# VIDILabs/open-volume-renderer

Measured on AMD Instinct MI355X. Metric: Msamples/s (primary ray-march samples after ERT); fps alongside, higher is better.
Workload: dtype f32

## Files before the change

open-volume-renderer_amd/csrc/host/frame.cpp:

```cpp
#include "state.hpp"

#include <cstdio>
#include <cstdlib>

namespace ovrhip {
namespace host {

static_assert(policy::kGeneral == LAYOUT_GENERAL && policy::kThin == LAYOUT_THIN && policy::kThinT == LAYOUT_THIN_T && policy::kQuad == LAYOUT_QUAD
              && policy::kLayoutCount == kLayouts && policy::kPoolSubCount == kPoolSubs, "policy.hpp restates ovr_hip_kernels.h");


static void shade_order_params(ovr_hip_renderer* r, PoolDesc& pd)
{
  const float beam = r->shade_beam;
  pd.order_grid = 0;
  if (!r->shade_order_on || !pd.order || !pd.order_key || !pd.order_ws) { pd.order = nullptr; return; }
  const RayMarchParams& P = r->P;
  const double diag = std::sqrt((double)r->vd.nx * r->vd.nx + (double)r->vd.ny * r->vd.ny + (double)r->vd.nz * r->vd.nz);
  const int G = diag <= 32.0 * beam ? 32 : diag <= 64.0 * beam ? 64 : 128;
  const double L[3] = { P.light.x, P.light.y, P.light.z };
  const int k = std::fabs(L[0]) <= std::fabs(L[1]) && std::fabs(L[0]) <= std::fabs(L[2]) ? 0 : std::fabs(L[1]) <= std::fabs(L[2]) ? 1 : 2;
  double U[3] = { 0, 0, 0 }, V[3];
  U[(k + 1) % 3] = L[(k + 2) % 3]; U[(k + 2) % 3] = -L[(k + 1) % 3];
  const double un = std::sqrt(U[0] * U[0] + U[1] * U[1] + U[2] * U[2]);
// ... 156 lines not shown
      HIP_TRY(hipMemsetAsync(r->d_grad[i], 0, n * 3 * sizeof(float), st));
    }
    if (f.recon_on) HIP_TRY(hipMemsetAsync(r->recon.d_count, 0, std::max<size_t>(n, 1) * sizeof(float), st));
  }
  r->frame_index++;
  return 0;
}

static void fill_target_params(ovr_hip_renderer* r, const FrameSetup& f)
{
  RayMarchParams& P = r->P;
  P.rgba = r->d_rgba[r->cur];
  nonzero_rect(r, r->d_rect[r->cur]);
  if (r->shard.current.world > 1 && r->group.members.size() <= 1) r->map_whole_set(r->cur);
  if (f.recon_on) r->map_whole_set(r->cur);
  r->recon.frame = f.recon_on;
  r->frame_set = r->cur;
  P.grad = r->d_grad[r->cur];
  P.accum = r->d_accum;
  P.width = r->fbsize.current.w;
  P.height = r->fbsize.current.h;
  P.frame_index = r->frame_index;
  P.accumulate = f.accumulate ? 1 : 0;
  P.spp = r->spp.current;
  P.shading = r->shading.current;
  P.step = 1.f / r->rate.current;
  P.base = 1.f;
  P.shadow_stride = (P.step * 10.f) * P.step;
  const float ex = r->spacing[0] * r->vd.nx, ey = r->spacing[1] * r->vd.ny, ez = r->spacing[2] * r->vd.nz;
  P.long_ray_steps = std::sqrt(ex * ex + ey * ey + ez * ez) / P.step;
}

static void choose_layout(ovr_hip_renderer* r, hipStream_t st)
{
  RayMarchParams& P = r->P;
  int choice = r->layout_choice.current;
  if (choice < 0) {
    const float dir[3] = { P.cam_dir.x, P.cam_dir.y, P.cam_dir.z }, inv_scale[3] = { P.inv_scale.x, P.inv_scale.y, P.inv_scale.z };
    choice = policy::layout_rule(dir, inv_scale);
  }
  const bool tune_l = r->layout_choice.current < 0, tune_p = r->pipeline.current == 0;
  const bool may_wait = !tune_l;
  if (choice < 0 || choice >= kLayouts || r->replica_state[choice] == 0) choice = LAYOUT_GENERAL;
  bool building = false;
  if (r->tune.on && (tune_l || tune_p) && r->tune.state == 1) {
    int states[kLayouts];
    for (int k = 0; k < kLayouts; ++k) states[k] = r->replica_state[k];
    const int wanted = r->tune.probe_build(tune_l, states);
    if (wanted >= 0) (void)start_replica_build(r, wanted, nullptr);
    building = poll_replica_builds(r) > 0;
    (void)hipGetLastError();
  }
  choice = r->tune.before_frame(choice, tune_l, tune_p, building);
  choice = resolve_layout(r, choice, may_wait, st);
  const float vs = P.vol.value_scale, vm = P.vol.value_min_clamp;
  P.vol = r->vd_replica[choice];
  P.vol.value_scale = vs;
  P.vol.value_min_clamp = vm;
  r->stats.layout = choice;
}

static void bind_general_layout(ovr_hip_renderer* r)
{
  RayMarchParams& P = r->P;
  const float vs = P.vol.value_scale, vm = P.vol.value_min_clamp;
  P.vol = r->vd_replica[LAYOUT_GENERAL];
  P.vol.value_scale = vs;
  P.vol.value_min_clamp = vm;
  r->stats.layout = LAYOUT_GENERAL;
  r->tune.frame = -1;
}

const float* projection_ranges(const ovr_hip_renderer* r) { return r->have_volume && r->mc_ranges_valid ? r->d_mc_minmax : nullptr; }

void fill_isosurface_params(const ovr_hip_renderer* r, RayMarchParams& q)
{
  const IsoP& p = r->isosurfaces.current;
  q.iso_n = p.n;
  for (int k = 0; k < OVR_HIP_MAX_ISOVALUES; ++k) q.iso_values[k] = k < p.n ? p.v[k] : 0.f;
}
static bool in_place_frame(const RayMarchParams& P) { return P.projection != OVR_HIP_PROJECT_OFF || P.iso_n > 0; }

static int fill_table_params(ovr_hip_renderer* r)
{
  RayMarchParams& P = r->P;
  P.tf_color = r->d_tf_color;
  P.tf_alpha = r->d_tf_alpha;
  P.n_color = r->n_color;
  P.n_alpha = r->n_alpha;
  P.rank = r->shard.current.rank;
  P.world = r->shard.current.world;
  P.tile_w = r->shard.current.tw;
  P.tile_h = r->shard.current.th;
  P.lds_staging = r->lds_staging.current;
  P.lds_brick_offset = 0;
  P.jitter_mode = r->jitter.current;
  P.jitter_noise = r->d_noise;
  P.jitter_xy = r->noise_xy;
  if (P.jitter_mode == 1 && !r->d_noise)
    return fail(OVR_HIP_ESTATE, "[hip] blue-noise pixel jitter enabled but no noise tile was set (ovr_hip_set_noise_tile)");
  P.counters = r->d_counters;
  P.majorant = nullptr;
  P.occupancy = nullptr;
  P.occupancy_fine = nullptr;
  P.projection = r->projection.current;
  P.mc_ranges = nullptr;
  fill_isosurface_params(r, P);
  return 0;
}

static int choose_skipping(ovr_hip_renderer* r, FrameSetup& f)
{
  RayMarchParams& P = r->P;
  if (in_place_frame(P)) {
    f.use_skip = false;
    if (r->skipping.current != 0) P.mc_ranges = projection_ranges(r);
  }
  else f.use_skip = r->skip.before_frame(r->skipping.current != 0, r->mc_majorant_valid);
  if (f.use_skip) {
    if (int e = update_macrocells(r, f.st)) return e;
    P.majorant = r->d_mc_majorant;
    P.occupancy = r->d_mc_occupancy;
// ... 266 lines not shown
  f.recon_on = r->reconstruction.current == OVR_HIP_RECONSTRUCT_FILL && f.sparse && r->shard.current.world <= 1 && r->group.members.size() <= 1 && !r->group.leader;
  if (f.recon_on)
    if (int e = ensure_reconstruction(r)) return e;
  if (int e = reset_accumulation(r, f)) return e;
  fill_target_params(r, f);
  if (r->projection.current != OVR_HIP_PROJECT_OFF || r->isosurfaces.current.n > 0) bind_general_layout(r);
  else choose_layout(r, st);
  if (int e = fill_table_params(r)) return e;
  if (int e = choose_skipping(r, f)) return e;
  r->P.shadow_lattice = nullptr;
  if (!in_place_frame(r->P) && r->P.shading == OVR_HIP_SHADE_FULL && r->shadow.current.mode != OVR_HIP_SHADOWS_MARCHED)
    if (int e = ensure_shadow_cache(r, r->P, st)) return e;
  f.conv_on = r->convergence.current.mode != OVR_HIP_CONVERGENCE_OFF && f.accumulate && !f.sparse;
  r->P.accum_half = nullptr;
  r->P.conv_asked = nullptr;
  if (f.conv_on) {
    if (int e = ensure_convergence(r, false)) return e;
    r->P.accum_half = r->conv.d_accum_half;
  }
  if (!f.sparse)
    if (int e = schedule_blocks(r, f)) return e;
  if (int e = prepare_convergence(r, f)) return e;
  if (r->conv.resolve_only) return launch_frame(r);
  if (f.sparse)
    if (int e = launch_frame_mask(r, f)) return e;
  if (int e = prepare_pool(r, f)) return e;
  return launch_frame(r);
}

static int launch_frame(ovr_hip_renderer* r)
{
  hipStream_t st = r->stream();
  const bool resolve = r->P.accum_half && r->convergence.current.mode == OVR_HIP_CONVERGENCE_ADAPTIVE && r->conv.retired > 0;
  const int blocks_x = (r->fbsize.current.w + 7) / 8;
  if (r->conv.resolve_only) {
    HIP_TRY(hipEventRecord(r->ev[0], st));
    HIP_TRY(launch_resolve_blocks(r->P, r->conv.d_lists + r->conv.list_cap, r->conv.retired, r->conv.d_frames, r->conv.d_grad_keep, blocks_x, st));
    HIP_TRY(hipEventRecord(r->ev[3], st));
    std::memset(r->h_counters, 0, 8 * sizeof(unsigned long long));
    r->frame_phase_timed = false;
    r->async_pending = true;
    return 0;
  }
  if (resolve) HIP_TRY(launch_resolve_blocks(r->P, r->conv.d_lists + r->conv.list_cap, r->conv.retired, r->conv.d_frames, r->conv.d_grad_keep, blocks_x, st));
  r->P.publish = r->h_counters;
  r->P.reduce_done = reinterpret_cast<unsigned int*>(reinterpret_cast<char*>(r->d_counters) + 128 + (size_t)kPoolCtrlWords * sizeof(unsigned int));
  r->P.zero_first = r->frame_words_dirty ? 1 : 0;
  if (r->frame_words_dirty) HIP_TRY(hipMemsetAsync(r->P.reduce_done, 0, sizeof(unsigned int), st));
  if (r->frame_words_dirty && r->pool.order_ws) HIP_TRY(hipMemsetAsync(r->pool.order_ws, 0, (size_t)kOrderWsWords * sizeof(unsigned int), st));
  r->frame_words_dirty = true;
  const bool phases = r->phase_timing.load();
  hipEvent_t evs[4] = { r->ev[0], phases ? r->ev[1] : nullptr, phases ? r->ev[2] : nullptr, r->ev[3] };
  r->frame_phase_timed = phases;
  r->plan = plan_raymarch(r->P);
  HIP_TRY(launch_raymarch(r->P, r->plan, st, evs));
  r->frame_words_dirty = false;
  if (r->conv.frame) {
    ConvergenceParams c{};
    c.accum = r->d_accum; c.accum_half = r->conv.d_accum_half; c.grad = r->P.grad; c.grad_keep = r->conv.d_grad_keep;
    c.width = r->P.width; c.height = r->P.height; c.frame_index = r->P.frame_index;
    c.rank = r->P.rank; c.world = r->P.world; c.tile_w = r->P.tile_w; c.tile_h = r->P.tile_h;
    c.blocks_x = blocks_x;
    c.adaptive = r->convergence.current.mode == OVR_HIP_CONVERGENCE_ADAPTIVE ? 1 : 0;
    c.threshold = r->convergence.current.threshold;
    c.sorted = r->conv.sorted; c.n_work = r->sched.n_work;
    c.active = r->P.schedule; c.n_active = r->P.n_schedule;
    c.active_out = r->conv.d_lists; c.retired_out = r->conv.d_lists ? r->conv.d_lists + r->conv.list_cap : nullptr;
    c.counts = r->conv.d_lists ? r->conv.d_lists + 2 * r->conv.list_cap : nullptr;
    c.block_error = r->conv.d_error; c.block_frames = r->conv.d_frames; c.words = r->conv.d_words;
    c.sub_capacity = r->P.pool.reqs ? r->P.pool.sub_capacity : 0xffffffffu;
    c.publish = r->conv.h_publish;
    r->conv.h_publish[3] = 0u;
    HIP_TRY(launch_convergence(c, st));
  }
  if (r->recon.frame) {
    ReconParams& c = r->recon.params;
    c = ReconParams{};
    c.width = r->P.width; c.height = r->P.height;
    (void)recon_plan(c);
    c.rgba = r->P.rgba; c.grad = r->P.grad;
    c.count = r->recon.d_count;
    c.accum = r->P.accumulate ? r->d_accum : nullptr;
    c.grad_sum = r->P.accumulate ? r->recon.d_grad : nullptr;
    c.pyramid = r->recon.d_pyramid;
    c.words = r->recon.d_words;
    c.sub_capacity = r->P.pool.reqs ? r->P.pool.sub_capacity : 0xffffffffu;
    c.publish = r->recon.h_publish;
    c.frame_index = r->P.frame_index;
    r->recon.h_publish[1] = 0u;
    r->recon.timed = phases;
    if (phases) HIP_TRY(hipEventRecord(r->recon.ev[0], st));
    HIP_TRY(launch_recon_scatter(c, r->recon.d_count, r->P.accumulate ? r->recon.d_grad : nullptr, r->P.sparse_xy, r->P.sparse_count, st));
    HIP_TRY(launch_reconstruct(c, st));
    if (phases) HIP_TRY(hipEventRecord(r->recon.ev[1], st));
  }
  r->async_pending = true;
  return 0;
}

static int resolve_pool(ovr_hip_renderer* r)
{
  if (r->P.pool.reqs) {
    auto asked = [&]() { return (size_t)r->h_ctrl[32 * (kPoolSubs + 1)]; };
    if (asked() > r->pool.sub_capacity && r->packed_early) r->stats.stale_tiles = 1;
    for (int attempt = 0; attempt < 4 && asked() > r->pool.sub_capacity; ++attempt) {
      if (int e = ensure_pool(r, policy::pool_grown(asked()))) return e;
      r->P.pool = r->pool;
      shade_order_params(r, r->P.pool);
// ... 165 lines not shown
```

open-volume-renderer_amd/csrc/host/launch_plan.hpp:

```cpp
#pragma once

#include <algorithm>
#include <cstddef>

namespace ovrhip {

constexpr int kBlock = 256;
constexpr int kWaves = kBlock / 64;
constexpr int request_queue_entries(int shade, bool pooled) { return shade == 0 ? 0 : (pooled ? 128 : 256); }
template <int SHADE, bool POOLED> struct QCfg {
  static constexpr int K = POOLED ? 4 : (SHADE == 0 ? 4 : 3);
  static constexpr int QCAP = request_queue_entries(SHADE, POOLED);
};
constexpr int kShadeReqBytes = 32;
constexpr int kLdsBrickCap = 384;
constexpr int kLdsRegionBytes = 32;
constexpr int kShadeBlocks = 1024;
constexpr unsigned int kDeepMaxBlocks = 10000;
constexpr int kCounterWords = 8;
constexpr int kAxisAbExtra = 3, kAxisZExtra = 2;

constexpr bool row_load_layout(int elem_bytes, bool quad) { return elem_bytes <= 2 && !quad; }
constexpr bool march_variant_exists(int shade, int am, bool pooled, bool skip, bool lds_staged, bool deep, bool material, bool clipped, bool f32_general,
                                    bool cached = false)
{
  if (cached && !(shade == 1 && material && !pooled)) return false;
  if (shade < 0 || shade > 2 || am < 0 || am > 4 || (f32_general && am == 4)) return false;
  if (pooled && shade == 0) return false;
  if (lds_staged) return f32_general && shade == 0 && !skip && am <= 1 && !deep && !material && !clipped;
  if (deep) return pooled && !skip && (am <= 1 || am == 4) && !material && !clipped;
  if (material && (shade == 0 || pooled)) return false;
  if (clipped && !pooled && material != (shade != 0)) return false;
  return true;
}
constexpr bool shade_variant_exists(int shade, int am, bool skip, bool material, bool clipped, bool cached = false)
{
  if (shade < 1 || shade > 2 || am < 0 || am > 4) return false;
  if (cached && !(shade == 1 && material)) return false;
  (void)skip;
  return !clipped || (shade == 2 && material);
}

constexpr int kProjectMaximum = 1, kProjectMinimum = 2, kProjectMean = 3;
constexpr int kProjectK = 4;
constexpr bool project_variant_exists(int mode, int am, bool skip, bool clipped)
{
  (void)clipped;
  if (mode < kProjectMaximum || mode > kProjectMean || am < 0 || am > 4) return false;
  return !skip || mode != kProjectMean;
}

constexpr int kMaxIsovalues = 4;
constexpr bool isosurface_variant_exists(int shade, int am, bool skip, bool clipped)
{
  (void)skip; (void)clipped;
  return shade >= 0 && shade <= 2 && am >= 0 && am <= 4;
}

constexpr size_t tf_lds_bytes(int n_color, int n_alpha)
{
  const size_t need = (size_t)n_color * 16 + (size_t)n_alpha * 4 + 32;
  return need <= 96 * 1024 ? need : 0;
}
constexpr size_t axis_table_bytes(int nx, int ny, int nz, int am)
{
  const size_t ab = (size_t)(nx + ny + kAxisAbExtra), ez = (size_t)(nz + kAxisZExtra);
  return am == 3 ? 0 : am == 2 ? ez * 8 + ab * 4 : (ab + ez) * 4;
}
constexpr size_t align16(size_t n) { return (n + 15) & ~(size_t)15; }

constexpr int addressing_mode(unsigned long long stored_bytes, int elem_bytes, int nx, int ny, int nz, int n_color, int n_alpha)
{
  const int am = stored_bytes <= 0x100000000ull ? 0 : (stored_bytes / (unsigned long long)elem_bytes < 0xffffffffull) ? 1 : 2;
  const size_t tables = axis_table_bytes(nx, ny, nz, am);
  const size_t fixed = tf_lds_bytes(n_color, n_alpha) + (size_t)kWaves * request_queue_entries(1, false) * kShadeReqBytes + 1024;
  return ((am == 2 && tables > 64 * 1024) || tables + 16 + fixed > 160 * 1024) ? 3 : am;
}

struct LaunchFacts {
  int elem_bytes = 4;
  bool quad = false, f32_general = false;
  int nx = 1, ny = 1, nz = 1;
  unsigned long long stored_bytes = 0;
  bool tables = true;
  int n_color = 1, n_alpha = 1, shading = 0;
  bool pool = false, skipping = false, sparse = false;
  unsigned long long sparse_hint_pixels = 0;
  int world = 1;
  unsigned int n_blocks_owned = 0, n_schedule = 0;
  bool schedule = true;
  bool clip_on = false, lds_staging = false;
  int row_loads = 0;
  int shade_blocks = 0;
  bool reference_material = true, shade_order = false;
  bool shadow_cache = false;
  int projection = 0;
  bool ranges = false;
  int isosurfaces = 0;
};
struct LaunchOverrides { int addressing = -1, deep = -1, shade_blocks = 0; };

struct LaunchPlan {
  int shading = 0;
  int am = 0;
  bool pooled = false, skip = false;
  struct March { bool lds_staged = false, deep = false, material = false, clipped = false; } march;
  struct Shade { bool material = false, clipped = false; } shade;
  bool shade_order = false;
  bool cached = false;
  struct Project { int mode = 0; bool skip = false, clipped = false; size_t lds_bytes = 0; } project;
  struct Isosurface { bool on = false, skip = false, clipped = false; size_t lds_bytes = 0; } isosurface;
  size_t march_lds_bytes = 0, shade_lds_bytes = 0;
  unsigned int lds_brick_offset = 0;
  int shade_grid_blocks = 0;
  bool error = false;
};

inline bool deep_rounds_pay(const LaunchFacts& f, const LaunchOverrides& o)
{
  if (o.deep >= 0) return o.deep != 0;
  if (f.sparse) return f.world == 1 && f.sparse_hint_pixels > 0 && f.sparse_hint_pixels <= 64ull * kDeepMaxBlocks;
  return f.world > 1 && f.n_blocks_owned <= kDeepMaxBlocks;
}

inline LaunchPlan plan_projection(const LaunchFacts& f, const LaunchOverrides& o)
{
  LaunchPlan pl;
  int am = addressing_mode(f.stored_bytes, f.elem_bytes, f.nx, f.ny, f.nz, f.n_color, f.n_alpha);
  if (o.addressing >= 0) am = std::min(std::max(am, o.addressing), 3);
  if (f.projection < kProjectMaximum || f.projection > kProjectMean || f.quad || (am < 3 && !f.tables) || (!f.sparse && f.n_schedule > 0 && !f.schedule)) {
    pl.error = true;
    return pl;
  }
  if (row_load_layout(f.elem_bytes, f.quad) && am == 0 && (f.row_loads > 0 ? f.row_loads != 1 : f.stored_bytes > (128ull << 20))) am = 4;
  pl.am = am;
  pl.project.mode = f.projection;
  pl.project.skip = f.ranges && f.projection != kProjectMean;
  pl.project.clipped = f.clip_on;
  pl.project.lds_bytes = std::max<size_t>(align16(axis_table_bytes(f.nx, f.ny, f.nz, am)), (size_t)kWaves * kCounterWords * 4);
  pl.march_lds_bytes = pl.project.lds_bytes;
  return pl;
}

inline LaunchPlan plan_isosurface(const LaunchFacts& f, const LaunchOverrides& o)
{
  LaunchPlan pl;
  int am = addressing_mode(f.stored_bytes, f.elem_bytes, f.nx, f.ny, f.nz, f.n_color, f.n_alpha);
  if (o.addressing >= 0) am = std::min(std::max(am, o.addressing), 3);
  if (f.isosurfaces < 1 || f.isosurfaces > kMaxIsovalues || f.quad || (am < 3 && !f.tables) || (!f.sparse && f.n_schedule > 0 && !f.schedule)) {
    pl.error = true;
    return pl;
  }
  if (row_load_layout(f.elem_bytes, f.quad) && am == 0 && (f.row_loads > 0 ? f.row_loads != 1 : f.stored_bytes > (128ull << 20))) am = 4;
  pl.am = am;
  pl.shading = f.shading == 0 || f.shading == 1 ? f.shading : 2;
  pl.isosurface.on = true;
  pl.isosurface.skip = f.ranges;
  pl.isosurface.clipped = f.clip_on;
  pl.isosurface.lds_bytes = std::max<size_t>(align16(axis_table_bytes(f.nx, f.ny, f.nz, am)), (size_t)kWaves * kCounterWords * 4);
  pl.march_lds_bytes = pl.isosurface.lds_bytes;
  return pl;
}

inline LaunchPlan plan_launch(const LaunchFacts& f, const LaunchOverrides& o = LaunchOverrides())
{
  if (f.isosurfaces != 0) return plan_isosurface(f, o);
  if (f.projection != 0) return plan_projection(f, o);
  LaunchPlan pl;
  pl.shading = f.shading == 0 || f.shading == 1 ? f.shading : 2;
  pl.cached = pl.shading == 2 && f.shadow_cache;
  if (pl.cached) pl.shading = 1;
  const int sh = pl.shading;
  int am = addressing_mode(f.stored_bytes, f.elem_bytes, f.nx, f.ny, f.nz, f.n_color, f.n_alpha);
  if (o.addressing >= 0) am = std::min(std::max(am, o.addressing), 3);
  const size_t tf = tf_lds_bytes(f.n_color, f.n_alpha);
  if ((am < 3 && !f.tables) || tf == 0 || (!f.sparse && f.n_schedule > 0 && !f.schedule)) { pl.error = true; return pl; }
  if (row_load_layout(f.elem_bytes, f.quad) && am == 0 && (f.row_loads > 0 ? f.row_loads != 1 : f.stored_bytes > (128ull << 20))) am = 4;
  pl.am = am;
  pl.skip = f.skipping;
  pl.pooled = sh != 0 && f.pool;
  const size_t tables = align16(axis_table_bytes(f.nx, f.ny, f.nz, am));
  const size_t queues = (size_t)kWaves * request_queue_entries(sh, pl.pooled) * kShadeReqBytes;
  if (!pl.pooled) {
    pl.march_lds_bytes = std::max<size_t>(tf + tables + queues, (size_t)kWaves * kCounterWords * 4);
    if (f.f32_general && sh == 0 && !f.skipping && am <= 1 && f.lds_staging && !f.sparse && !f.clip_on) {
      pl.march.lds_staged = true;
      pl.lds_brick_offset = (unsigned int)align16(pl.march_lds_bytes);
      pl.march_lds_bytes = pl.lds_brick_offset + (size_t)kLdsBrickCap * 128 + kLdsRegionBytes + 12 * 4 + 2 * 4 + 16;
    }
    else {
      pl.march.clipped = f.clip_on;
      pl.march.material = sh != 0 && (f.clip_on || !f.reference_material || pl.cached);
    }
    return pl;
  }
  pl.march_lds_bytes = queues + tables + (size_t)f.n_alpha * 4 + 64;
  pl.march.clipped = f.clip_on;
  pl.march.deep = !f.skipping && (am <= 1 || am == 4) && !f.clip_on && deep_rounds_pay(f, o);
  pl.shade.clipped = sh == 2 && f.clip_on;
  pl.shade.material = pl.shade.clipped || !f.reference_material || pl.cached;
  pl.shade_order = sh == 2 && f.shade_order;
  pl.shade_lds_bytes = std::max<size_t>(tf + tables, 64);
  const int blocks = o.shade_blocks > 0 ? o.shade_blocks : f.shade_blocks;
  pl.shade_grid_blocks = blocks > 0 ? std::min(blocks, kShadeBlocks) : kShadeBlocks;
  return pl;
}

}
```

open-volume-renderer_amd/csrc/host/state.hpp:

```cpp
#pragma once

#include "../../../include/ovr_hip.h"
#include "../ovr_hip_kernels.h"
#include "../ovr_hip_update.h"
#pragma GCC visibility push(hidden)
#include "commit_plan.hpp"
#include "policy.hpp"
#pragma GCC visibility pop

#include <hip/hip_runtime.h>

#include <algorithm>
#include <atomic>
#include <cmath>
#include <cstdint>
#include <cstring>
#include <functional>
#include <mutex>
#include <string>
#include <thread>
#include <vector>

struct ovr_hip_renderer;
struct GroupWorker;
// ... 115 lines not shown
  bool shipped_by_rccl = false;
  float* d_payload[2] = { nullptr, nullptr };
  float* d_gather[2] = { nullptr, nullptr };
  size_t payload_floats[2] = { 0, 0 }, stride[2] = { 0, 0 };
  int fb[5] = { 0, 0, 0, 0, 0 };
  bool grad = true;
  void* rccl_comm = nullptr;
  ovr_hip_stats own_stats{};
  double gather_ms = 0.0;
  double upload_ms = 0.0;
  double update_ms = 0.0;
  GroupWorker* worker = nullptr;
  hipEvent_t ev_gathered = nullptr;
  bool broken = false;
  std::string broken_why;
  double host_us[4] = { 0, 0, 0, 0 };
};

}
}

struct ovr_hip_renderer {
  template <typename T> using Queued = ovrhip::host::Queued<T>;
  int device = 0;
  std::mutex mtx;
  hipStream_t own_stream[2] = { nullptr, nullptr };
  hipStream_t user_stream = nullptr;
  bool use_user_stream = false;
  hipEvent_t ev[4] = { nullptr, nullptr, nullptr, nullptr };

  Queued<ovrhip::host::Size2> fbsize;
  Queued<ovrhip::host::CameraP> camera;
  Queued<ovrhip::host::TfnP> tfn;
  Queued<ovrhip::host::FocusP> focus;
  Queued<int> spp, sparse, accumulate, shading, grid_convention, pipeline, skipping, jitter, lds_staging;
  Queued<int> projection;
  bool projection_skipped = false;
  Queued<ovrhip::host::IsoP> isosurfaces;
  bool isosurface_skipped = false;
  Queued<float> rate;
  Queued<ovrhip::host::ShardP> shard;
  Queued<ovrhip::host::LightP> light;
  Queued<ovrhip::host::MaterialP> material;
  Queued<ovrhip::host::ClipP> clip;
  Queued<ovrhip::host::ShadowP> shadow;
  Queued<ovrhip::host::ConvP> convergence;
  Queued<int> reconstruction;
  Queued<int> layouts;
  Queued<int> layout_choice;

  void* d_volume = nullptr;
  std::atomic<size_t> volume_bytes{ 0 };
  ovrhip::VolumeDesc vd{};
  void* d_replica[ovrhip::kLayouts] = {};
  void* d_axis[ovrhip::kLayouts] = {};
  ovrhip::VolumeDesc vd_replica[ovrhip::kLayouts] = {};
  std::atomic<int> replica_state[ovrhip::kLayouts] = {};
  std::thread builder[ovrhip::kLayouts];
  hipStream_t build_stream = nullptr;
  hipEvent_t build_ev[ovrhip::kLayouts] = {};
  int value_type = 0;
  float origin[3] = { 0, 0, 0 }, spacing[3] = { 1, 1, 1 };
  bool have_volume = false;
  float data_lower = 0.f, data_upper = 0.f;
  float* d_data_range = nullptr;
  double upload_ms[4] = { 0, 0, 0, 0 };
  void* d_update_stage = nullptr;
  size_t update_stage_bytes = 0;
  double update_ms[4] = { 0, 0, 0, 0 };

  ovrhip::policy::Tuner tune;
  ovrhip::policy::AutoPipeline auto_pipe;
  ovrhip::policy::Skip skip;
  bool shade_order_on = true;
  float shade_beam = 32.f;

  float* d_mc_minmax = nullptr;
  float* d_mc_majorant = nullptr;
  unsigned char* d_mc_occupancy = nullptr;
  unsigned char* d_mc_fine = nullptr;
  size_t mc_cells = 0;
  bool mc_ranges_valid = false, mc_majorant_valid = false;

  float* d_tf_color = nullptr;
  float* d_tf_alpha = nullptr;
  float* h_tf = nullptr;
  hipEvent_t ev_tf = nullptr;
  bool tf_copy_pending = false;
  int n_color = 0, n_alpha = 0;
  bool have_tfn = false;

  float* d_rgba[2] = { nullptr, nullptr };
  float* d_grad[2] = { nullptr, nullptr };
  float* h_rgba[2] = { nullptr, nullptr };
  float* h_grad[2] = { nullptr, nullptr };
  int h_rgba_rect[2][4] = {}, h_grad_rect[2][4] = {};
  int d_rect[2][4] = {};
  float* d_accum = nullptr;
  uint32_t* d_rgba8 = nullptr;
  uint32_t* h_rgba8 = nullptr;
  uint16_t* d_rgba16f = nullptr;
  uint16_t* h_rgba16f = nullptr;
  float* d_spp_rgba = nullptr;
  float* d_spp_grad = nullptr;
  size_t fb_pixels = 0;
  int cur = 0;
  bool fb_reset = true;
  int frame_index = 0;
  bool camera_dirty = true;

  ovrhip::host::ConvergenceState conv;
  ovrhip::host::ReconstructionState recon;
  ovrhip::host::ShadowCacheState shadow_cache;

  float* d_noise = nullptr;
  int noise_xy = 0;
  int32_t* d_sparse_xy = nullptr;
  unsigned int* d_block_counts = nullptr;
  unsigned long long* d_sparse_count = nullptr;
  size_t sparse_pixels = 0;
  unsigned long long sparse_prev_pixels = 0;

  unsigned long long* d_counters = nullptr;
  std::atomic<bool> phase_timing{ true };
  bool frame_phase_timed = true;
  bool frame_words_dirty = true;
  unsigned int* d_block_counters = nullptr;
// ... 81 lines not shown
```

open-volume-renderer_amd/csrc/host/update_extent.hpp:

```cpp
#pragma once

#include <algorithm>
#include <cstdint>

namespace ovrhip {
namespace update {

struct Box { int lo[3], hi[3]; };

struct Geometry { int cx, mbx, by, bz; bool transposed, quad; int lx, ly, lz; };

enum { kOk = 0, kNull = 1, kMemKind = 2, kType = 3, kExtent = 4, kOutside = 5 };
inline int check_arguments(const void* data, const int32_t* lower, const int32_t* extent, int mem_kind, int value_type, int resident_type, const int dims[3])
{
  if (!data || !lower || !extent) return kNull;
  if (mem_kind != 0 && mem_kind != 1) return kMemKind;
  if (value_type != resident_type) return kType;
  for (int k = 0; k < 3; ++k)
    if (extent[k] < 1) return kExtent;
  for (int k = 0; k < 3; ++k)
    if (lower[k] < 0 || lower[k] >= dims[k] || extent[k] > dims[k] - lower[k]) return kOutside;
  return kOk;
}
inline const char* check_text(int rule)
{
  switch (rule) {
  case kNull: return "null argument";
  case kMemKind: return "bad mem_kind";
  case kType: return "value_type is not the resident volume's";
  case kExtent: return "extent must be positive";
  case kOutside: return "the box leaves the grid";
  default: return "";
  }
}

struct BrickRange {
  int brick_lo, brick_hi;
  int macro_lo, macro_hi;
  int row_lo, row_hi;
  int layer_lo, layer_hi;
};

inline void pair_axis_bricks(int cx, int na, int bricks_total, int a, int b, int& lo, int& hi)
{
  const int p_lo = a == 0 ? 0 : a + 1;
  lo = p_lo == 0 ? 0 : (p_lo - 1) / cx;
  hi = b == na ? bricks_total - 1 : std::min(b / cx, bricks_total - 1);
}

inline BrickRange brick_range(const Geometry& g, const int dims[3], int macros_a, const Box& box)
{
  const int ia = g.transposed ? 1 : 0, ib = g.transposed ? 0 : 1;
  BrickRange r;
  pair_axis_bricks(g.cx, dims[ia], macros_a * g.mbx, box.lo[ia], box.hi[ia], r.brick_lo, r.brick_hi);
  r.macro_lo = r.brick_lo / g.mbx; r.macro_hi = r.brick_hi / g.mbx;
  r.row_lo = box.lo[ib] >> 5; r.row_hi = (box.hi[ib] - 1) >> 5;
  r.layer_lo = box.lo[2] >> g.bz; r.layer_hi = (box.hi[2] - 1) >> g.bz;
  return r;
}

struct QuadRange {
  int u_lo, u_hi, v_lo, v_hi;
  int macro_lo, macro_hi;
  int row_lo, row_hi;
  int layer_lo, layer_hi;
};
inline QuadRange quad_range(const Geometry& g, const Box& box)
{
  QuadRange r;
  r.u_lo = box.lo[0]; r.u_hi = box.hi[0];
  r.v_lo = box.lo[1]; r.v_hi = box.hi[1];
  r.macro_lo = r.u_lo >> 5; r.macro_hi = r.u_hi >> 5;
  r.row_lo = r.v_lo >> 5; r.row_hi = r.v_hi >> 5;
  r.layer_lo = box.lo[2] >> g.lz; r.layer_hi = (box.hi[2] - 1) >> g.lz;
  return r;
}

inline void macrocell_axis(int n, int a, int b, int& lo, int& hi)
{
  const int cells = (n + 15) / 16;
  lo = a <= 16 ? 0 : a >> 4;
  hi = std::min(b >> 4, cells - 1);
}
struct CellRange { int lo[3], hi[3]; };
inline CellRange macrocell_range(const int dims[3], const Box& box)
{
  CellRange c;
  for (int k = 0; k < 3; ++k) macrocell_axis(dims[k], box.lo[k], box.hi[k], c.lo[k], c.hi[k]);
  return c;
}

}
}
```

open-volume-renderer_amd/csrc/host/volume.cpp:

```cpp
#include "state.hpp"

#include <cfloat>
#include <chrono>
#include <cstdlib>

using namespace ovrhip;
using namespace ovrhip::host;

namespace ovrhip {
namespace host {

static float integer_normalize(float value, int type)
{
  switch (type) {
  case OVR_HIP_TYPE_UINT8: return (float)(uint8_t)value / 255.f;
  case OVR_HIP_TYPE_INT8: { const float n = (float)(int8_t)value / 127.f; return n < -1.f ? -1.f : n; }
  case OVR_HIP_TYPE_UINT16: return (float)(uint16_t)value / 65535.f;
  case OVR_HIP_TYPE_INT16: { const float n = (float)(int16_t)value / 32767.f; return n < -1.f ? -1.f : n; }
  case OVR_HIP_TYPE_UINT32: return (float)(uint32_t)value / (float)UINT32_MAX;
  case OVR_HIP_TYPE_INT32: { const float n = (float)(int32_t)value / (float)INT32_MAX; return n < -1.f ? -1.f : n; }
  default: return value;
  }
}
static int device_value_type(int t)
// ... 159 lines not shown
  for (int i = 0; i < na; ++i) a[i] = t.alphas[2 * i + 1];
  HIP_TRY(hipMemcpyAsync(r->d_tf_color, r->h_tf, words * sizeof(float), hipMemcpyHostToDevice, r->stream()));
  if (!r->ev_tf) HIP_TRY(hipEventCreateWithFlags(&r->ev_tf, hipEventDisableTiming));
  HIP_TRY(hipEventRecord(r->ev_tf, r->stream()));
  r->tf_copy_pending = true;
  r->have_tfn = true;
  return 0;
}

static int update_macrocell_ranges(ovr_hip_renderer* r, hipStream_t st)
{
  const size_t cells = (size_t)((r->vd.nx + 15) / 16) * ((r->vd.ny + 15) / 16) * ((r->vd.nz + 15) / 16);
  if (cells != r->mc_cells || !r->d_mc_minmax) {
    HIP_TRY(hipDeviceSynchronize());
    if (r->d_mc_minmax) HIP_TRY(hipFree(r->d_mc_minmax));
    if (r->d_mc_majorant) HIP_TRY(hipFree(r->d_mc_majorant));
    if (r->d_mc_occupancy) HIP_TRY(hipFree(r->d_mc_occupancy));
    if (r->d_mc_fine) HIP_TRY(hipFree(r->d_mc_fine));
    r->d_mc_fine = nullptr;
    r->d_mc_minmax = r->d_mc_majorant = nullptr;
    r->d_mc_occupancy = nullptr;
    r->mc_cells = 0;
    HIP_TRY(hipMalloc((void**)&r->d_mc_minmax, cells * 2 * sizeof(float)));
    HIP_TRY(hipMalloc((void**)&r->d_mc_majorant, cells * sizeof(float)));
    HIP_TRY(hipMalloc((void**)&r->d_mc_occupancy, cells));
    HIP_TRY(hipMalloc((void**)&r->d_mc_fine, cells));
    r->mc_cells = cells;
    r->mc_ranges_valid = r->mc_majorant_valid = false;
  }
  if (!r->mc_ranges_valid) {
    VolumeDesc vd = r->vd;
    vd.data = r->d_volume;
    HIP_TRY(launch_macrocell_ranges(vd, r->d_mc_minmax, st));
    r->mc_ranges_valid = true;
    r->mc_majorant_valid = false;
  }
  return 0;
}

int update_macrocells(ovr_hip_renderer* r, hipStream_t st)
{
  if (int e = update_macrocell_ranges(r, st)) return e;
  const size_t cells = r->mc_cells;
  if (!r->mc_majorant_valid) {
    HIP_TRY(launch_macrocell_majorants(r->d_mc_minmax, (unsigned int)cells, r->d_tf_alpha, r->n_alpha, r->P.tf_lower, r->P.tf_upper, r->d_mc_majorant, st));
    HIP_TRY(launch_macrocell_coarse(r->d_mc_majorant, r->vd.nx, r->vd.ny, r->vd.nz, r->d_mc_occupancy, r->d_mc_fine, st));
    r->mc_majorant_valid = true;
  }
  return 0;
}

void join_builders(ovr_hip_renderer* r)
{
  for (int k = 0; k < kLayouts; ++k)
    if (r->builder[k].joinable()) r->builder[k].join();
}

static void drop_replica(ovr_hip_renderer* r, int k)
{
  if (k == LAYOUT_GENERAL) return;
  if (r->builder[k].joinable()) r->builder[k].join();
  if (r->d_replica[k]) { (void)hipFree(r->d_replica[k]); r->volume_bytes -= (size_t)r->vd_replica[k].bytes; }
  if (r->d_axis[k]) (void)hipFree(r->d_axis[k]);
  r->d_replica[k] = nullptr; r->d_axis[k] = nullptr;
  r->replica_state[k] = 0;
}

static void build_replica_host(ovr_hip_renderer* r, int k, std::string* err)
{
  (void)hipSetDevice(r->device);
  VolumeDesc t = r->vd_replica[k];
  void *d_data = nullptr, *d_tab = nullptr;
  hipError_t e = hipMalloc(&d_data, (size_t)t.bytes + 64);
  if (e == hipSuccess) e = hipMalloc(&d_tab, axis_table_bytes(t));
  if (e == hipSuccess) {
    t.data = d_data;
    if (getenv("OVR_HIP_POISON_ALLOC") && atoi(getenv("OVR_HIP_POISON_ALLOC")) != 0) e = hipMemsetAsync(d_data, 0xff, (size_t)t.bytes, r->build_stream);
    if (e == hipSuccess) e = hipMemsetAsync((char*)d_data + (size_t)t.bytes, 0, 64, r->build_stream);
  }
  if (e == hipSuccess) e = launch_axis_tables(t, d_tab, r->build_stream);
  if (e == hipSuccess) {
    VolumeDesc g = r->vd_replica[LAYOUT_GENERAL];
    g.data = r->d_volume;
    e = launch_rebrick(g, d_data, t, r->build_stream);
  }
  if (e == hipSuccess) e = hipEventRecord(r->build_ev[k], r->build_stream);
  if (e != hipSuccess) {
    (void)hipGetLastError();
    (void)hipStreamSynchronize(r->build_stream);
    if (err) *err = hipGetErrorString(e);
    if (d_data) (void)hipFree(d_data);
    if (d_tab) (void)hipFree(d_tab);
    r->replica_state[k].store(0, std::memory_order_release);
    return;
  }
  r->vd_replica[k] = t;
  r->d_replica[k] = d_data;
  r->d_axis[k] = d_tab;
  r->volume_bytes += (size_t)t.bytes;
  r->replica_state[k].store(2, std::memory_order_release);
}

int start_replica_build(ovr_hip_renderer* r, int k, std::string* err, bool background)
{
  int planned = 1;
  if (!r->replica_state[k].compare_exchange_strong(planned, 4)) return 0;
  if (r->builder[k].joinable()) r->builder[k].join();
  static const bool threads = !(getenv("OVR_HIP_BUILD_THREAD") && atoi(getenv("OVR_HIP_BUILD_THREAD")) == 0);
  bool started = false;
  if (background && threads) {
    try { r->builder[k] = std::thread(build_replica_host, r, k, nullptr); started = true; }
    catch (const std::exception&) { started = false; }
  }
  if (!started) build_replica_host(r, k, err);
  return 0;
}

int resolve_layout(ovr_hip_renderer* r, int choice, bool may_wait, hipStream_t st)
{
  if (choice <= LAYOUT_GENERAL || choice >= kLayouts || r->replica_state[choice].load(std::memory_order_acquire) == 0) return LAYOUT_GENERAL;
  if (r->replica_state[choice] == 1) (void)start_replica_build(r, choice, nullptr, !may_wait);
  if (r->replica_state[choice] == 4 && may_wait && r->builder[choice].joinable()) r->builder[choice].join();
  int state = r->replica_state[choice].load(std::memory_order_acquire);
  if (state == 2 && hipEventQuery(r->build_ev[choice]) == hipSuccess) { r->replica_state[choice] = 3; state = 3; }
  if (state == 3) return choice;
  if (state == 2 && may_wait && hipStreamWaitEvent(st, r->build_ev[choice], 0) == hipSuccess) return choice;
  (void)hipGetLastError();
  return LAYOUT_GENERAL;
}
int poll_replica_builds(ovr_hip_renderer* r)
{
  int building = 0;
  for (int k = 1; k < kLayouts; ++k) {
    int state = r->replica_state[k].load(std::memory_order_acquire);
    if (state == 2 && hipEventQuery(r->build_ev[k]) == hipSuccess) { r->replica_state[k] = 3; state = 3; }
    if (state == 2 || state == 4) building++;
  }
  return building;
}

static double ms_since(std::chrono::high_resolution_clock::time_point t0) { return std::chrono::duration<double, std::milli>(std::chrono::high_resolution_clock::now() - t0).count(); }

static int plan_replicas(ovr_hip_renderer* r, int vt, const VolumeDesc& vd)
{
  {
    std::lock_guard<std::mutex> lk(r->mtx);
    (void)r->layouts.update();
  }
  {
    size_t free_b = 0, total_b = 0;
    HIP_TRY(hipMemGetInfo(&free_b, &total_b));
    double planned = 0.0;
    auto plan = [&](int k, VolumeDesc& t) { t = vd; t.data = nullptr; t.axis_ab = nullptr; t.axis_z = nullptr; return volume_layout(replica_voxel_type(vt, k), vd.nx, vd.ny, vd.nz, t); };
    if (r->layouts.current != 0 && replica_voxel_type(vt, LAYOUT_THIN) >= 0) {
      VolumeDesc t1, t2;
      if (plan(LAYOUT_THIN, t1) && plan(LAYOUT_THIN_T, t2) && layout_offsets_fit(t1) && layout_offsets_fit(t2) && (r->layouts.current == 2 || (double)(t1.bytes + t2.bytes) <= 0.4 * (double)free_b)) {
        r->vd_replica[LAYOUT_THIN] = t1; r->vd_replica[LAYOUT_THIN_T] = t2;
        r->replica_state[LAYOUT_THIN] = r->replica_state[LAYOUT_THIN_T] = 1;
        planned += (double)(t1.bytes + t2.bytes);
      }
      else if (r->layouts.current == 2) return fail(OVR_HIP_EINVAL, "[hip] volume replicas requested (layouts mode 2) but one z layer of a thin replica exceeds 2^32 elements");
    }
    static const bool want_quad = !(getenv("OVR_HIP_QUAD") && atoi(getenv("OVR_HIP_QUAD")) == 0);
    if (want_quad && r->layouts.current != 0 && replica_voxel_type(vt, LAYOUT_QUAD) >= 0) {
      VolumeDesc tq;
      if (plan(LAYOUT_QUAD, tq) && layout_offsets_fit(tq) && (r->layouts.current == 2 || (double)tq.bytes + planned <= 0.4 * (double)free_b)) {
        r->vd_replica[LAYOUT_QUAD] = tq;
        r->replica_state[LAYOUT_QUAD] = 1;
      }
    }
  }
  return 0;
}

struct UploadTimes { double alloc = 0.0, copy = 0.0, kern = 0.0; };

static int upload_voxels(ovr_hip_renderer* r, const void* data, int mem_kind, int value_type, std::chrono::high_resolution_clock::time_point t_seg, UploadTimes& t)
{
  const VolumeDesc& vd = r->vd_replica[0];
  hipStream_t st = r->own_stream[0];
  auto relayout_all = [&](const void* src, int z0, int nzc) -> hipError_t {
    return launch_relayout(src, value_type, r->d_replica[0], r->vd_replica[0], z0, nzc, st);
  };

  const size_t in_es = value_type_size(value_type);
  const size_t slice_bytes = (size_t)vd.nx * vd.ny * in_es;
  int src_device = r->device;
  if (mem_kind == OVR_HIP_MEM_DEVICE) {
    hipPointerAttribute_t attr{};
    if (hipPointerGetAttributes(&attr, data) == hipSuccess) src_device = attr.device;
    else (void)hipGetLastError();
  }
  if (mem_kind == OVR_HIP_MEM_DEVICE && src_device == r->device) {
    for (int z0 = 0; z0 < vd.nz; z0 += 32768) {
      const int nzc = std::min(32768, vd.nz - z0);
      HIP_TRY(relayout_all((const char*)data + (size_t)z0 * slice_bytes, z0, nzc));
    }
    HIP_TRY(hipStreamSynchronize(st));
    t.kern += ms_since(t_seg);
  }
  else {
    size_t slab = std::max<size_t>(1, ((size_t)1 << 30) / std::max<size_t>(1, slice_bytes));
    slab = std::min<size_t>(slab, (size_t)vd.nz);
    void* d_stage = nullptr;
    t_seg = std::chrono::high_resolution_clock::now();
    HIP_TRY(hipMalloc(&d_stage, slab * slice_bytes));
    t.alloc += ms_since(t_seg);
    for (int z0 = 0; z0 < vd.nz; z0 += (int)slab) {
      const int nzc = (int)std::min<size_t>(slab, (size_t)(vd.nz - z0));
      t_seg = std::chrono::high_resolution_clock::now();
      hipError_t e = mem_kind == OVR_HIP_MEM_DEVICE
                         ? hipMemcpyPeerAsync(d_stage, r->device, (const char*)data + (size_t)z0 * slice_bytes, src_device, (size_t)nzc * slice_bytes, st)
                         : hipMemcpyAsync(d_stage, (const char*)data + (size_t)z0 * slice_bytes, (size_t)nzc * slice_bytes, hipMemcpyHostToDevice, st);
      if (e == hipSuccess) e = hipStreamSynchronize(st);
      t.copy += ms_since(t_seg);
      t_seg = std::chrono::high_resolution_clock::now();
      if (e == hipSuccess) e = relayout_all(d_stage, z0, nzc);
      if (e == hipSuccess) e = hipStreamSynchronize(st);
      t.kern += ms_since(t_seg);
      if (e != hipSuccess) { (void)hipFree(d_stage); return fail(OVR_HIP_EDEVICE, std::string("[hip] volume upload failed: ") + hipGetErrorString(e)); }
    }
    HIP_TRY(hipFree(d_stage));
  }
  return 0;
}

static int set_volume_one(ovr_hip_renderer* r, const void* data, int mem_kind, int value_type, const int32_t dims[3],
                          const float grid_origin[3], const float grid_spacing[3])
{
  const auto t_call = std::chrono::high_resolution_clock::now();
  UploadTimes t;
  if (!r || !data || !dims || !grid_origin || !grid_spacing) return fail(OVR_HIP_EINVAL, "[hip] ovr_hip_set_volume: null argument");
  for (double& v : r->upload_ms) v = 0.0;
  if (dims[0] < 1 || dims[1] < 1 || dims[2] < 1) return fail(OVR_HIP_EINVAL, "[hip] ovr_hip_set_volume: dims must be positive");
  const int vt = device_voxel_type(value_type);
  if (vt < 0) return fail(OVR_HIP_EINVAL, "[Optix7] unexpected volume type ...");
  if (mem_kind != OVR_HIP_MEM_HOST && mem_kind != OVR_HIP_MEM_DEVICE) return fail(OVR_HIP_EINVAL, "[hip] ovr_hip_set_volume: bad mem_kind");
  if (int e = set_device(r)) return e;
  if (int e = finish_frame_one(r)) return e;
  HIP_TRY(hipDeviceSynchronize());

  hipStream_t st = r->own_stream[0];
  VolumeDesc vd{};
  if (!volume_layout(vt, dims[0], dims[1], dims[2], vd)) return fail(OVR_HIP_EINVAL, "[hip] ovr_hip_set_volume: no layout for this voxel type");
  vd.value_scale = 1.f;
  vd.value_min_clamp = -FLT_MAX;
  if (vt == VOX_U8) vd.value_scale = 1.f / 255.f;
  if (vt == VOX_I8) { vd.value_scale = 1.f / 127.f; vd.value_min_clamp = -127.f; }
  const size_t bytes = (size_t)vd.bytes;
  if (!layout_offsets_fit(vd))
    return fail(OVR_HIP_EINVAL, "[hip] ovr_hip_set_volume: one z layer of the volume exceeds 2^32 stored voxels (x * y too large for the 32-bit in-plane offsets)");

  auto t_seg = std::chrono::high_resolution_clock::now();
  join_builders(r);
  HIP_TRY(hipStreamSynchronize(r->build_stream));
  for (int k = 0; k < kLayouts; ++k) {
    if (r->d_replica[k]) HIP_TRY(hipFree(r->d_replica[k]));
    r->d_replica[k] = nullptr;
    if (r->d_axis[k]) HIP_TRY(hipFree(r->d_axis[k]));
    r->d_axis[k] = nullptr;
    r->vd_replica[k] = VolumeDesc{};
    r->replica_state[k] = 0;
  }
  r->d_volume = nullptr;
  r->have_volume = false;
  HIP_TRY(hipMalloc(&r->d_replica[0], bytes + 64));
  if (getenv("OVR_HIP_POISON_ALLOC") && atoi(getenv("OVR_HIP_POISON_ALLOC")) != 0) HIP_TRY(hipMemsetAsync(r->d_replica[0], 0xff, bytes, st));
  HIP_TRY(hipMemsetAsync((char*)r->d_replica[0] + bytes, 0, 64, st));
  r->d_volume = r->d_replica[0];
  r->volume_bytes = bytes;
  vd.data = r->d_volume;
  r->vd_replica[0] = vd;
  r->replica_state[0] = 3;
  if (int e = plan_replicas(r, vt, vd)) return e;
  HIP_TRY(hipMalloc(&r->d_axis[0], axis_table_bytes(r->vd_replica[0])));
  t.alloc += ms_since(t_seg);
  t_seg = std::chrono::high_resolution_clock::now();
  HIP_TRY(launch_axis_tables(r->vd_replica[0], r->d_axis[0], st));
  vd = r->vd_replica[0];
  if (int e = upload_voxels(r, data, mem_kind, value_type, t_seg, t)) return e;
  t_seg = std::chrono::high_resolution_clock::now();
  r->vd = vd;
  if (r->layouts.current == 2) {
    for (int k = 1; k < kLayouts; ++k) {
      if (r->replica_state[k] != 1) continue;
      std::string err;
      (void)start_replica_build(r, k, &err, false);
      if (r->replica_state[k] != 2) {
        for (int j = 1; j < kLayouts; ++j) drop_replica(r, j);
        return fail(OVR_HIP_EDEVICE, std::string("[hip] volume replicas requested (layouts mode 2) but their allocation failed: ") + err);
      }
    }
    HIP_TRY(hipStreamSynchronize(r->build_stream));
    for (int k = 1; k < kLayouts; ++k)
      if (r->replica_state[k] == 2) r->replica_state[k] = 3;
  }
  r->value_type = value_type;
  std::memcpy(r->origin, grid_origin, sizeof(r->origin));
  std::memcpy(r->spacing, grid_spacing, sizeof(r->spacing));
  r->have_volume = true;
  {
    commit::Changes ch;
    ch.happened(commit::kVolumeUpload);
    commit::CommitFacts facts;
    facts.volume = true;
    apply_effects(r, commit::plan_commit(ch, facts));
  }
  if (int e = update_macrocell_ranges(r, st)) return e;
  HIP_TRY(launch_minmax_reduce(r->d_mc_minmax, (unsigned long long)r->mc_cells, r->d_data_range, st));
  float dr[2] = { 0.f, 0.f };
  HIP_TRY(hipMemcpyAsync(dr, r->d_data_range, sizeof(dr), hipMemcpyDeviceToHost, st));
  HIP_TRY(hipStreamSynchronize(st));
  r->data_lower = dr[0];
  r->data_upper = dr[1];
  r->P.tf_lower = dr[0];
  r->P.tf_upper = dr[1];
  update_tfn_range(r);
  t.kern += ms_since(t_seg);
  r->upload_ms[0] = ms_since(t_call); r->upload_ms[1] = t.alloc; r->upload_ms[2] = t.copy; r->upload_ms[3] = t.kern;
  return 0;
}

static int update_volume_one(ovr_hip_renderer* r, const void* data, int mem_kind, int value_type, const int32_t lower[3], const int32_t extent[3])
{
  const auto t_call = std::chrono::high_resolution_clock::now();
  UploadTimes t;
  for (double& v : r->update_ms) v = 0.0;
  if (int e = set_device(r)) return e;
  if (int e = finish_frame_one(r)) return e;
  hipStream_t st = r->own_stream[0];
  update::Box box;
  for (int k = 0; k < 3; ++k) { box.lo[k] = lower[k]; box.hi[k] = lower[k] + extent[k]; }

  join_builders(r);
  for (int k = 1; k < kLayouts; ++k)
    if (r->replica_state[k].load(std::memory_order_acquire) == 2) HIP_TRY(hipStreamWaitEvent(st, r->build_ev[k], 0));

  const size_t in_es = value_type_size(value_type);
  const size_t slice_bytes = (size_t)extent[0] * (size_t)extent[1] * in_es;
  int src_device = r->device;
  if (mem_kind == OVR_HIP_MEM_DEVICE) {
    hipPointerAttribute_t attr{};
    if (hipPointerGetAttributes(&attr, data) == hipSuccess) src_device = attr.device;
    else (void)hipGetLastError();
  }
  const bool direct = mem_kind == OVR_HIP_MEM_DEVICE && src_device == r->device;
  size_t slab = (size_t)extent[2];
  if (!direct) {
    slab = std::min<size_t>(std::max<size_t>(1, ((size_t)1 << 30) / std::max<size_t>(1, slice_bytes)), (size_t)extent[2]);
    if (r->update_stage_bytes < slab * slice_bytes) {
      const auto t_seg = std::chrono::high_resolution_clock::now();
      if (r->d_update_stage) HIP_TRY(hipFree(r->d_update_stage));
      r->d_update_stage = nullptr; r->update_stage_bytes = 0;
      HIP_TRY(hipMalloc(&r->d_update_stage, slab * slice_bytes));
      r->update_stage_bytes = slab * slice_bytes;
      t.alloc += ms_since(t_seg);
    }
  }
  auto write = [&]() -> int {
    for (int z0 = 0; z0 < extent[2]; z0 += (int)slab) {
      const int nzc = (int)std::min<size_t>(slab, (size_t)(extent[2] - z0));
      const void* src = (const char*)data + (size_t)z0 * slice_bytes;
      auto t_seg = std::chrono::high_resolution_clock::now();
      if (!direct) {
        HIP_TRY(mem_kind == OVR_HIP_MEM_DEVICE ? hipMemcpyPeerAsync(r->d_update_stage, r->device, src, src_device, (size_t)nzc * slice_bytes, st)
                                               : hipMemcpyAsync(r->d_update_stage, src, (size_t)nzc * slice_bytes, hipMemcpyHostToDevice, st));
        HIP_TRY(hipStreamSynchronize(st));
        t.copy += ms_since(t_seg);
        t_seg = std::chrono::high_resolution_clock::now();
        src = r->d_update_stage;
      }
      update::Box part = box;
      part.lo[2] = box.lo[2] + z0; part.hi[2] = part.lo[2] + nzc;
      HIP_TRY(launch_update_general(src, value_type, r->d_replica[0], r->vd_replica[0], part, st));
      if (!direct) HIP_TRY(hipStreamSynchronize(st));
      t.kern += ms_since(t_seg);
    }
    const auto t_seg = std::chrono::high_resolution_clock::now();
    VolumeDesc g = r->vd_replica[LAYOUT_GENERAL];
    g.data = r->d_volume;
    for (int k = 1; k < kLayouts; ++k) {
      const int state = r->replica_state[k].load(std::memory_order_acquire);
      if (state == 2 || state == 3) HIP_TRY(launch_update_replica(g, r->d_replica[k], r->vd_replica[k], box, st));
    }
    const int dims[3] = { r->vd.nx, r->vd.ny, r->vd.nz };
    VolumeDesc vd = r->vd;
    vd.data = r->d_volume;
    HIP_TRY(launch_macrocell_ranges_box(vd, r->d_mc_minmax, update::macrocell_range(dims, box), st));
    HIP_TRY(launch_minmax_reduce(r->d_mc_minmax, (unsigned long long)r->mc_cells, r->d_data_range, st));
    float dr[2] = { 0.f, 0.f };
    HIP_TRY(hipMemcpyAsync(dr, r->d_data_range, sizeof(dr), hipMemcpyDeviceToHost, st));
    HIP_TRY(hipStreamSynchronize(st));
    r->data_lower = dr[0];
    r->data_upper = dr[1];
    r->P.tf_lower = dr[0];
    r->P.tf_upper = dr[1];
    update_tfn_range(r);
    t.kern += ms_since(t_seg);
    return 0;
  };
  if (!r->d_mc_minmax || !r->mc_ranges_valid) return fail(OVR_HIP_ESTATE, "[hip] ovr_hip_update_volume: the resident volume has no macrocell ranges");
  if (int e = write()) {
    r->have_volume = false;
    return e;
  }
  commit::Changes ch;
  ch.happened(commit::kVolumeUpdate);
  commit::CommitFacts facts;
  facts.volume = true;
  apply_effects(r, commit::plan_commit(ch, facts));
  r->update_ms[0] = ms_since(t_call); r->update_ms[1] = t.alloc; r->update_ms[2] = t.copy; r->update_ms[3] = t.kern;
  return 0;
}

}
}

extern "C" {

int ovr_hip_update_volume(ovr_hip_renderer* r, const void* data, int mem_kind, int value_type, const int32_t lower[3], const int32_t extent[3])
{
  if (!r) return fail(OVR_HIP_EINVAL, "[hip] ovr_hip_update_volume: null argument");
  if (!r->have_volume && data && lower && extent) return fail(OVR_HIP_ESTATE, "[hip] ovr_hip_update_volume: no volume is set");
  const int dims[3] = { r->vd.nx, r->vd.ny, r->vd.nz };
  if (const int rule = update::check_arguments(data, lower, extent, mem_kind, value_type, r->value_type, dims))
    return fail(OVR_HIP_EINVAL, std::string("[hip] ovr_hip_update_volume: ") + update::check_text(rule));
  if (r->group.members.size() <= 1) return update_volume_one(r, data, mem_kind, value_type, lower, extent);
  const auto t0 = std::chrono::high_resolution_clock::now();
  if (int e = set_device(r)) return e;
  if (int e = finish_frame(r)) return e;
  const int e = group_call(r, [=](ovr_hip_renderer* m) { return update_volume_one(m, data, mem_kind, value_type, lower, extent); },
                           [&] { return update_volume_one(r, data, mem_kind, value_type, lower, extent); });
  if (e) {
    const std::string msg = g_last_error;
// ... 81 lines not shown
```

open-volume-renderer_amd/csrc/ovr_hip_api.cpp:

```cpp
#include "host/state.hpp"

#include <chrono>
#include <cstdio>
#include <cstdlib>

using namespace ovrhip;
using namespace ovrhip::host;

#define GROUP_FORWARD(r, call)                                                                                          \
  do {                                                                                                                  \
    for (size_t i_ = 1; i_ < (r)->group.members.size(); ++i_) {                                                         \
      ovr_hip_renderer* m = (r)->group.members[i_];                                                                     \
      if (int e_ = (call)) { (void)hipSetDevice((r)->device); return e_; }                                              \
    }                                                                                                                   \
    if ((r)->group.members.size() > 1) (void)hipSetDevice((r)->device);                                                 \
  } while (0)

extern "C" {

const char* ovr_hip_last_error(void) { return g_last_error.c_str(); }
int ovr_hip_abi_version(void) { return OVR_HIP_ABI_VERSION; }

int ovr_hip_create(ovr_hip_renderer** out, int device_id)
{
  if (!out) return fail(OVR_HIP_EINVAL, "[hip] ovr_hip_create: null output pointer");
  *out = nullptr;
  int count = 0;
  if (hipGetDeviceCount(&count) != hipSuccess || count <= 0)
    return fail(OVR_HIP_EDEVICE, "[hip] no HIP device available - this backend has no CPU fallback");
  if (device_id < 0 || device_id >= count) return fail(OVR_HIP_EINVAL, "[hip] invalid device ordinal " + std::to_string(device_id));
  HIP_TRY(hipSetDevice(device_id));
  hipDeviceProp_t prop;
  HIP_TRY(hipGetDeviceProperties(&prop, device_id));
  if (std::string(prop.gcnArchName).find("gfx950") == std::string::npos)
    return fail(OVR_HIP_EDEVICE, std::string("[hip] device is ") + prop.gcnArchName + ", this library is built for gfx950 (MI355X) only");
  ovr_hip_renderer* r = new ovr_hip_renderer();
  r->device = device_id;
  apply_lighting(r);
  apply_clip_box(r);
  auto acquire = [&]() -> int {
    HIP_TRY(hipStreamCreate(&r->own_stream[0]));
    HIP_TRY(hipStreamCreate(&r->own_stream[1]));
    for (int i = 0; i < 4; ++i) HIP_TRY(hipEventCreate(&r->ev[i]));
    {
      int lo = 0, hi = 0;
      if (hipDeviceGetStreamPriorityRange(&lo, &hi) != hipSuccess) { (void)hipGetLastError(); lo = hi = 0; }
      HIP_TRY(hipStreamCreateWithPriority(&r->build_stream, hipStreamNonBlocking, hi));
    }
    for (int k = 0; k < kLayouts; ++k) HIP_TRY(hipEventCreateWithFlags(&r->build_ev[k], hipEventDisableTiming));
    HIP_TRY(hipMalloc((void**)&r->d_counters, kFrameWordsBytes));
    HIP_TRY(hipMemset(r->d_counters, 0, kFrameWordsBytes));
    HIP_TRY(hipMalloc((void**)&r->d_sparse_count, sizeof(unsigned long long)));
    HIP_TRY(hipMalloc((void**)&r->d_data_range, minmax_reduce_floats() * sizeof(float)));
    HIP_TRY(hipHostMalloc((void**)&r->h_counters, 8 * sizeof(unsigned long long) + (size_t)kPoolCtrlWords * sizeof(unsigned int), hipHostMallocDefault));
    r->h_ctrl = reinterpret_cast<unsigned int*>(r->h_counters + 8);
    return 0;
  };
  if (int e = acquire()) { ovr_hip_destroy(r); return e; }
  std::memset(r->h_counters, 0, 8 * sizeof(unsigned long long) + (size_t)kPoolCtrlWords * sizeof(unsigned int));
  r->spp.init(1);
  r->sparse.init(0);
  r->accumulate.init(0);
  r->shading.init(OVR_HIP_SHADE_FULL);
  r->grid_convention.init(OVR_HIP_GRID_CELL_CENTRED);
  r->rate.init(1.f);
  r->layouts.init(1);
  r->layout_choice.init(-1);
  if (const char* f = getenv("OVR_HIP_LAYOUTS")) r->layouts.init(atoi(f));
  if (const char* f = getenv("OVR_HIP_SKIP_ADAPTIVE")) r->skip.adaptive = atoi(f) != 0;
  if (const char* f = getenv("OVR_HIP_TUNE")) r->tune.on = atoi(f) != 0;
  if (const char* f = getenv("OVR_HIP_SHADE_ORDER")) r->shade_order_on = atoi(f) != 0;
  if (const char* f = getenv("OVR_HIP_ROW_LOADS")) r->P.row_loads = atoi(f) != 0 ? 2 : 1;
  if (const char* f = getenv("OVR_HIP_SHADE_BEAM")) r->shade_beam = std::max(1.f, (float)atof(f));
  *out = r;
  return 0;
}
void ovr_hip_destroy(ovr_hip_renderer* r)
{
  if (!r) return;
  if (r->group.members.size() > 1) group_stop_workers(r);
  for (size_t i = 1; i < r->group.members.size(); ++i) ovr_hip_destroy(r->group.members[i]);
  r->group.members.clear();
  join_builders(r);
  (void)hipSetDevice(r->device);
  (void)hipDeviceSynchronize();
  group_release(r);
  (void)free_framebuffers(r);
  for (int k = 0; k < kLayouts; ++k) {
    if (r->d_replica[k]) (void)hipFree(r->d_replica[k]);
    if (r->d_axis[k]) (void)hipFree(r->d_axis[k]);
  }
  if (r->d_tf_color) (void)hipFree(r->d_tf_color);
  if (r->h_tf) (void)hipHostFree(r->h_tf);
  if (r->ev_tf) (void)hipEventDestroy(r->ev_tf);
  if (r->d_noise) (void)hipFree(r->d_noise);
  if (r->d_mc_minmax) (void)hipFree(r->d_mc_minmax);
  if (r->d_mc_majorant) (void)hipFree(r->d_mc_majorant);
  if (r->d_mc_occupancy) (void)hipFree(r->d_mc_occupancy);
  if (r->d_mc_fine) (void)hipFree(r->d_mc_fine);
  if (r->d_counters) (void)hipFree(r->d_counters);
  if (r->d_sparse_count) (void)hipFree(r->d_sparse_count);
  if (r->d_data_range) (void)hipFree(r->d_data_range);
  if (r->d_update_stage) (void)hipFree(r->d_update_stage);
  free_shadow_cache(r);
  if (r->h_counters) (void)hipHostFree(r->h_counters);
  if (r->conv.h_publish) (void)hipHostFree(r->conv.h_publish);
  if (r->recon.h_publish) (void)hipHostFree(r->recon.h_publish);
  for (int i = 0; i < 2; ++i) if (r->recon.ev[i]) (void)hipEventDestroy(r->recon.ev[i]);
  for (int i = 0; i < 4; ++i) if (r->ev[i]) (void)hipEventDestroy(r->ev[i]);
  if (r->pool.reqs) (void)hipFree(r->pool.reqs);
  if (r->pool.chunk_next) (void)hipFree(r->pool.chunk_next);
  if (r->pool.chunk_n) (void)hipFree(r->pool.chunk_n);
  if (r->pool.shade_counters) (void)hipFree(r->pool.shade_counters);
  if (r->pool.order) (void)hipFree(r->pool.order);
  if (r->pool.order_key) (void)hipFree(r->pool.order_key);
  if (r->pool.order_ws) (void)hipFree(r->pool.order_ws);

  if (r->d_block_counters) (void)hipFree(r->d_block_counters);
  if (r->sched.h_info) (void)hipHostFree(r->sched.h_info);
  if (r->d_trace) (void)hipFree(r->d_trace);
  for (int i = 0; i < 2; ++i)
    if (r->own_stream[i]) (void)hipStreamDestroy(r->own_stream[i]);
  if (r->build_stream) (void)hipStreamDestroy(r->build_stream);
  for (int k = 0; k < kLayouts; ++k)
    if (r->build_ev[k]) (void)hipEventDestroy(r->build_ev[k]);
  delete r;
}

int ovr_hip_set_stream(ovr_hip_renderer* r, void* s)
{
  if (!r) return fail(OVR_HIP_EINVAL, "[hip] null renderer");
  if (r->group.members.size() > 1 && s) return fail(OVR_HIP_EINVAL, "[hip] ovr_hip_set_stream: a device group renders on one stream per device");
  if (int e = finish_frame(r)) return e;
  HIP_TRY(hipStreamSynchronize(r->stream()));
  for (int i = 0; i < 2; ++i) HIP_TRY(hipStreamSynchronize(r->own_stream[i]));
  r->user_stream = (hipStream_t)s;
  r->use_user_stream = (s != nullptr);
  return 0;
}
int ovr_hip_set_phase_timing(ovr_hip_renderer* r, int32_t on)
{
  if (!r) return fail(OVR_HIP_EINVAL, "[hip] null renderer");
  GroupLock gl(r);
  r->phase_timing.store(on != 0);
  GROUP_FORWARD(r, ovr_hip_set_phase_timing(m, on));
  return 0;
}

int ovr_hip_set_grid_convention(ovr_hip_renderer* r, int c)
{
  if (!r) return fail(OVR_HIP_EINVAL, "[hip] null renderer");
  if (c != OVR_HIP_GRID_CELL_CENTRED && c != OVR_HIP_GRID_VERTEX_CENTRED) return fail(OVR_HIP_EINVAL, "[hip] unknown grid convention");
  GroupLock gl(r);
  { std::lock_guard<std::mutex> lk(r->mtx); r->grid_convention.set(c); }
  GROUP_FORWARD(r, ovr_hip_set_grid_convention(m, c));
  return 0;
}

int ovr_hip_set_transfer_function(ovr_hip_renderer* r, const float* colors, int32_t n_colors, const float* alphas, int32_t n_alphas,
                                  float lo, float hi)
{
  if (!r) return fail(OVR_HIP_EINVAL, "[hip] null renderer");
  if (n_colors < 0 || n_alphas < 0 || (n_colors > 0 && !colors) || (n_alphas > 0 && !alphas))
    return fail(OVR_HIP_EINVAL, "[hip] ovr_hip_set_transfer_function: bad arguments");
  GroupLock gl(r);
  {
    std::lock_guard<std::mutex> lk(r->mtx);
    TfnP t;
    t.colors.assign(colors, colors + (size_t)n_colors * 3);
    t.alphas.assign(alphas, alphas + (size_t)n_alphas * 2);
    t.lo = lo;
    t.hi = hi;
    r->tfn.set(t);
  }
  GROUP_FORWARD(r, ovr_hip_set_transfer_function(m, colors, n_colors, alphas, n_alphas, lo, hi));
  return 0;
}
// ... 1046 lines not shown
```

open-volume-renderer_amd/csrc/ovr_hip_device.h:

```cpp
#pragma once
#include "ovr_hip_kernels.h"

#include <float.h>
#include <math.h>
#include <stdlib.h>
#include <algorithm>

namespace ovrhip {

struct f3 { float x, y, z; };
__device__ __forceinline__ f3 mk3(float x, float y, float z) { f3 r; r.x = x; r.y = y; r.z = z; return r; }
__device__ __forceinline__ f3 ld3(const float3_& a) { return mk3(a.x, a.y, a.z); }
__device__ __forceinline__ float dot3(f3 a, f3 b) { return fmaf(a.x, b.x, fmaf(a.y, b.y, a.z * b.z)); }
__device__ __forceinline__ float clampf(float x, float lo, float hi) { return __builtin_amdgcn_fmed3f(x, lo, hi); }
__device__ __forceinline__ float clamp01(float x) { return fminf(fmaxf(x, 0.f), 1.f); }
__device__ __forceinline__ float lerpf(float a, float b, float f) { return fmaf(f, b - a, a); }
#ifndef OVR_PARITY_EXACT
#define OVR_PARITY_EXACT 0
#endif
__device__ __forceinline__ f3 normalize3(f3 v)
{
#if OVR_PARITY_EXACT
  const float l = sqrtf(dot3(v, v));
  return mk3(v.x / l, v.y / l, v.z / l);
#endif
  const float r = __builtin_amdgcn_rsqf(dot3(v, v));
  return mk3(v.x * r, v.y * r, v.z * r);
}
__device__ __forceinline__ f3 normalize3_exact(f3 v)
{
  const float l = sqrtf(dot3(v, v));
  return mk3(v.x / l, v.y / l, v.z / l);
}

__device__ __forceinline__ float det_log2f(float x)
{
  if (!(x > 0.f)) return x == 0.f ? -__builtin_inff() : __builtin_nanf("");
  if (x > 3.402823466e+38f) return x;
  unsigned int ix = __float_as_uint(x);
  int e = (int)(ix >> 23) - 127;
  if (e == -127) { ix = __float_as_uint(x * 8388608.f); e = (int)(ix >> 23) - 127 - 23; }
  float m = __uint_as_float((ix & 0x007fffffu) | 0x3f800000u);
  if (m > 0x1.6a09e6p+0f) { m = m * 0.5f; e += 1; }
  const float f = m - 1.f;
  float p = -0x1.b8f078p-4f;
  p = fmaf(p, f, 0x1.7aec18p-3f);
  p = fmaf(p, f, -0x1.881ca4p-3f);
  p = fmaf(p, f, 0x1.a37bc2p-3f);
  p = fmaf(p, f, -0x1.eab168p-3f);
  p = fmaf(p, f, 0x1.277a9ap-2f);
  p = fmaf(p, f, -0x1.715a9p-2f);
  p = fmaf(p, f, 0x1.ec70a8p-2f);
  p = fmaf(p, f, -0x1.71547p-1f);
  p = fmaf(p, f, 0x1.715476p+0f);
// ... 77 lines not shown
  static constexpr bool kQuad = false;
};
template <> struct Vox<VOX_U16_TT> : Vox<VOX_U16_T> { static constexpr bool kTransposed = true; };
template <> struct Vox<VOX_I16> {
  typedef short T; typedef i16x2_u P;
  static constexpr int cx = 3, mbx = 10, by = 2, bz = 2;
  static constexpr bool kScale = false, kClamp = false;
  static constexpr bool kTransposed = false;
  static constexpr bool kQuad = false;
};
template <> struct Vox<VOX_U8> {
  typedef unsigned char T; typedef u8x2_u P;
  static constexpr int cx = 7, mbx = 4, by = 2, bz = 2;
  static constexpr bool kScale = true, kClamp = false;
  static constexpr bool kTransposed = false;
  static constexpr bool kQuad = false;
};
template <> struct Vox<VOX_I8> {
  typedef signed char T; typedef i8x2_u P;
  static constexpr int cx = 7, mbx = 4, by = 2, bz = 2;
  static constexpr bool kScale = true, kClamp = true;
  static constexpr bool kTransposed = false;
  static constexpr bool kQuad = false;
};

typedef float f32x4_q __attribute__((ext_vector_type(4)));
typedef unsigned short u16x4_q __attribute__((ext_vector_type(4)));
typedef unsigned char u8x4_q __attribute__((ext_vector_type(4)));
template <> struct Vox<VOX_F32_Q> {
  typedef float T; typedef f32x2_u P; typedef f32x4_q Q;
  static constexpr int lx = 1, ly = 1, lz = 1;
  static constexpr int cx = 2, mbx = 16, by = 1, bz = 1;
  static constexpr bool kScale = false, kClamp = false;
  static constexpr bool kTransposed = false;
  static constexpr bool kQuad = true;
};
template <> struct Vox<VOX_U16_Q> {
  typedef unsigned short T; typedef u16x2_u P; typedef u16x4_q Q;
  static constexpr int lx = 2, ly = 1, lz = 1;
  static constexpr int cx = 4, mbx = 8, by = 1, bz = 1;
  static constexpr bool kScale = false, kClamp = false;
  static constexpr bool kTransposed = false;
  static constexpr bool kQuad = true;
};
template <> struct Vox<VOX_U8_Q> {
  typedef unsigned char T; typedef u8x2_u P; typedef u8x4_q Q;
  static constexpr int lx = 2, ly = 2, lz = 1;
  static constexpr int cx = 4, mbx = 8, by = 2, bz = 1;
  static constexpr bool kScale = true, kClamp = false;
  static constexpr bool kTransposed = false;
  static constexpr bool kQuad = true;
};

template <int VT> struct BrickMap {
  typedef Vox<VT> V;
  static constexpr unsigned SX = V::cx + 1;
  static constexpr unsigned BV = SX << (V::by + V::bz);
  static constexpr unsigned sby = V::mbx * BV, sbz = (32u >> V::by) * V::mbx * BV;
  static constexpr unsigned MV = (32u >> V::bz) * sbz;
  static constexpr unsigned MCX = V::cx * V::mbx;
  static_assert(BV * sizeof(typename V::T) == 128, "a brick is exactly one 128-byte L1/L2 line");
  static __host__ __device__ __forceinline__ unsigned div_cx(unsigned x) { return (unsigned)(((unsigned long long)x * ((0xffffffffull / V::cx) + 1ull)) >> 32); }
  static __host__ __device__ __forceinline__ unsigned div_mbx(unsigned b) { return (unsigned)(((unsigned long long)b * ((0xffffffffull / V::mbx) + 1ull)) >> 32); }
  static __host__ __device__ __forceinline__ unsigned X(unsigned x)
  {
    const unsigned b = div_cx(x), xr = x - b * V::cx;
    const unsigned m = div_mbx(b), bm = b - m * V::mbx;
    return xr + bm * BV + m * MV;
  }
  static __host__ __device__ __forceinline__ unsigned Y(unsigned y, unsigned macro_y_stride)
  {
    return (y & ((1u << V::by) - 1u)) * SX + ((y >> V::by) & ((32u >> V::by) - 1u)) * sby + (y >> 5) * macro_y_stride;
  }
  static __host__ __device__ __forceinline__ unsigned Zlo(unsigned z)
  {
    return ((z & ((1u << V::bz) - 1u)) << V::by) * SX + ((z >> V::bz) & ((32u >> V::bz) - 1u)) * sbz;
  }
};

template <int VT> struct QuadMap {
  typedef Vox<VT> V;
  static constexpr unsigned SX = 2, BV = 128u / (unsigned)sizeof(typename V::T);
  static constexpr unsigned MV = 32u * 32u * 32u * 4u, MCX = 32;
  static constexpr unsigned bx_ = 32u >> V::lx, by_ = 32u >> V::ly;
  static_assert((4u << (V::lx + V::ly + V::lz)) == BV, "a brick is exactly one 128-byte L1/L2 line");
  static __host__ __device__ __forceinline__ unsigned div_cx(unsigned x) { return x >> V::lx; }
  static __host__ __device__ __forceinline__ unsigned X(unsigned x) { return (x & ((1u << V::lx) - 1u)) * 4u + ((x >> V::lx) & (bx_ - 1u)) * BV + (x >> 5) * MV; }
  static __host__ __device__ __forceinline__ unsigned Y(unsigned y, unsigned macro_y_stride)
  {
    return (y & ((1u << V::ly) - 1u)) * (4u << V::lx) + ((y >> V::ly) & (by_ - 1u)) * (bx_ * BV) + (y >> 5) * macro_y_stride;
  }
  static __host__ __device__ __forceinline__ unsigned Zlo(unsigned z)
  {
    return (z & ((1u << V::lz) - 1u)) * (4u << (V::lx + V::ly)) + ((z >> V::lz) & ((32u >> V::lz) - 1u)) * (bx_ * by_ * BV);
  }
};
template <> struct BrickMap<VOX_F32_Q> : QuadMap<VOX_F32_Q> {};
template <> struct BrickMap<VOX_U16_Q> : QuadMap<VOX_U16_Q> {};
template <> struct BrickMap<VOX_U8_Q> : QuadMap<VOX_U8_Q> {};

struct VolConsts {
  const void* data;
  const unsigned int *tab_x, *tab_y, *tab_z;
  const unsigned long long* tab_z64;
  int nx1, ny1, nz1;
  const float* majorant;
  const unsigned char* occupancy;
  const unsigned char* occupancy_fine;
  int mcx1, mcy1, mcz1;
  unsigned int macro_y;
  unsigned long long macro_z;
  f3 cs, cb;
  float vscale, vmin;
};

__device__ __forceinline__ int floor_to_int(float x)
{
  int r;
  asm("v_cvt_flr_i32_f32 %0, %1" : "=v"(r) : "v"(x));
  return r;
}
__device__ __forceinline__ void axis_tap(float po, float cs, float cb, int& i0, float& f)
{
  const float p = clamp01(po);
  const float x = fmaf(p, cs, cb);
  f = __builtin_amdgcn_fractf(x);
  i0 = floor_to_int(x);
}

struct Tap {
  float c000, c100, c010, c110, c001, c101, c011, c111;
  float fx, fy, fz;
  int x0, y0, z0;
};


__device__ __forceinline__ void tap_coords(const VolConsts& vc, f3 p, Tap& t)
{
  axis_tap(p.x, vc.cs.x, vc.cb.x, t.x0, t.fx);
  axis_tap(p.y, vc.cs.y, vc.cb.y, t.y0, t.fy);
  axis_tap(p.z, vc.cs.z, vc.cb.z, t.z0, t.fz);
}

__device__ __forceinline__ unsigned int tap_cell(const VolConsts& vc, const Tap& t)
{
  const int cx = min((t.x0 + 1) >> 4, vc.mcx1), cy = min((t.y0 + 1) >> 4, vc.mcy1), cz = min((t.z0 + 1) >> 4, vc.mcz1);
  return (unsigned int)cx + (unsigned int)(vc.mcx1 + 1) * ((unsigned int)cy + (unsigned int)(vc.mcy1 + 1) * (unsigned int)cz);
}

// ... 7 lines not shown
    static_assert(BrickMap<VT>::SX * sizeof(T) <= 8, "row loads: a pair must not cross its aligned 8 bytes, so a brick row is at most 8 bytes");
    constexpr unsigned per = 8u / (unsigned)sizeof(B);
    const unsigned long long al = off & ~(unsigned long long)(per - 1u);
    const unsigned sh = ((unsigned)off & (per - 1u)) * (8u * (unsigned)sizeof(B));
    const uint2 row = *reinterpret_cast<const uint2*>(base + al);
    const unsigned w = (unsigned)((((unsigned long long)row.y << 32) | (unsigned long long)row.x) >> sh);
    P r;
    if constexpr (sizeof(T) == 2) { r.x = (T)(w & 0xffffu); r.y = (T)(w >> 16); }
    else { r.x = (T)(w & 0xffu); r.y = (T)((w >> 8) & 0xffu); }
    return r;
  }
  else return *reinterpret_cast<const P*>(base + off);
}

template <int VT, int AM>
__device__ __forceinline__ void tap_loads(const VolConsts& vc, Tap& t)
{
  typedef BrickMap<VT> M;
  typedef typename Vox<VT>::T T;
  typedef typename Vox<VT>::P P;
  if constexpr (Vox<VT>::kQuad) {
    typedef typename Vox<VT>::Q Q;
    Q q0, q1;
    if (AM == 3) {
      const unsigned z0 = (unsigned)max(t.z0, 0), z1 = (unsigned)min(t.z0 + 1, vc.nz1);
      const unsigned o = M::X((unsigned)(t.x0 + 1)) + M::Y((unsigned)(t.y0 + 1), vc.macro_y);
      const T* base = static_cast<const T*>(vc.data);
      const unsigned long long oz0 = (unsigned long long)M::Zlo(z0) + (unsigned long long)(z0 >> 5) * vc.macro_z;
      const unsigned long long oz1 = (unsigned long long)M::Zlo(z1) + (unsigned long long)(z1 >> 5) * vc.macro_z;
      q0 = *reinterpret_cast<const Q*>(base + (oz0 + o)); q1 = *reinterpret_cast<const Q*>(base + (oz1 + o));
    }
    else if (AM == 2) {
      const unsigned o = vc.tab_x[t.x0] + vc.tab_y[t.y0];
      const unsigned long long oz0 = vc.tab_z64[t.z0], oz1 = vc.tab_z64[t.z0 + 1];
      const T* base = static_cast<const T*>(vc.data);
      q0 = *reinterpret_cast<const Q*>(base + (oz0 + o)); q1 = *reinterpret_cast<const Q*>(base + (oz1 + o));
    }
    else {
      const unsigned o = vc.tab_x[t.x0] + vc.tab_y[t.y0];
      const unsigned oz0 = vc.tab_z[t.z0], oz1 = vc.tab_z[t.z0 + 1];
      if (AM == 1) {
        const T* base = static_cast<const T*>(vc.data);
        q0 = *reinterpret_cast<const Q*>(base + (oz0 + o)); q1 = *reinterpret_cast<const Q*>(base + (oz1 + o));
      }
      else {
        const char* cb = static_cast<const char*>(vc.data);
        q0 = *reinterpret_cast<const Q*>(cb + (oz0 + o)); q1 = *reinterpret_cast<const Q*>(cb + (oz1 + o));
      }
    }
    t.c000 = (float)q0.x; t.c100 = (float)q0.y; t.c010 = (float)q0.z; t.c110 = (float)q0.w;
    t.c001 = (float)q1.x; t.c101 = (float)q1.y; t.c011 = (float)q1.z; t.c111 = (float)q1.w;
    return;
  }
  constexpr bool TR = Vox<VT>::kTransposed;
  const int a0 = TR ? t.y0 : t.x0, b0 = TR ? t.x0 : t.y0, z0 = t.z0;
  P p00, p10, p01, p11;
  if (AM == 3) {
    const int nb1 = TR ? vc.nx1 : vc.ny1;
    const unsigned bc0 = (unsigned)max(b0, 0), bc1 = (unsigned)min(b0 + 1, nb1), zc0 = (unsigned)max(z0, 0), zc1 = (unsigned)min(z0 + 1, vc.nz1);
    const unsigned ox = M::X((unsigned)(a0 + 1));
    const unsigned o0 = ox + M::Y(bc0, vc.macro_y), o1 = ox + M::Y(bc1, vc.macro_y);
    const T* base = static_cast<const T*>(vc.data);
    const unsigned long long oz0 = (unsigned long long)M::Zlo(zc0) + (unsigned long long)(zc0 >> 5) * vc.macro_z;
    const unsigned long long oz1 = (unsigned long long)M::Zlo(zc1) + (unsigned long long)(zc1 >> 5) * vc.macro_z;
    p00 = *reinterpret_cast<const P*>(base + (oz0 + o0)); p10 = *reinterpret_cast<const P*>(base + (oz0 + o1));
    p01 = *reinterpret_cast<const P*>(base + (oz1 + o0)); p11 = *reinterpret_cast<const P*>(base + (oz1 + o1));
  }
  else if (AM == 2) {
    const unsigned ox = vc.tab_x[a0];
    const unsigned o0 = ox + vc.tab_y[b0], o1 = ox + vc.tab_y[b0 + 1];
    const unsigned long long oz0 = vc.tab_z64[z0], oz1 = vc.tab_z64[z0 + 1];
    const T* base = static_cast<const T*>(vc.data);
    p00 = load_pair<VT, AM>(base, oz0 + o0); p10 = load_pair<VT, AM>(base, oz0 + o1);
    p01 = load_pair<VT, AM>(base, oz1 + o0); p11 = load_pair<VT, AM>(base, oz1 + o1);
  }
  else {
    const unsigned ox = vc.tab_x[a0];
    const unsigned oy0 = vc.tab_y[b0], oy1 = vc.tab_y[b0 + 1];
    const unsigned oz0 = vc.tab_z[z0], oz1 = vc.tab_z[z0 + 1];
    const unsigned o0 = ox + oy0, o1 = ox + oy1;
    if (AM == 1) {
      const T* base = static_cast<const T*>(vc.data);
      p00 = load_pair<VT, AM>(base, (unsigned long long)(oz0 + o0)); p10 = load_pair<VT, AM>(base, (unsigned long long)(oz0 + o1));
      p01 = load_pair<VT, AM>(base, (unsigned long long)(oz1 + o0)); p11 = load_pair<VT, AM>(base, (unsigned long long)(oz1 + o1));
    }
    else {
      const char* cb = static_cast<const char*>(vc.data);
      p00 = load_pair<VT, AM>(cb, (unsigned long long)(oz0 + o0)); p10 = load_pair<VT, AM>(cb, (unsigned long long)(oz0 + o1));
      p01 = load_pair<VT, AM>(cb, (unsigned long long)(oz1 + o0)); p11 = load_pair<VT, AM>(cb, (unsigned long long)(oz1 + o1));
    }
  }
  if (!TR) {
    t.c000 = (float)p00.x; t.c100 = (float)p00.y; t.c010 = (float)p10.x; t.c110 = (float)p10.y;
    t.c001 = (float)p01.x; t.c101 = (float)p01.y; t.c011 = (float)p11.x; t.c111 = (float)p11.y;
  }
  else {
    t.c000 = (float)p00.x; t.c010 = (float)p00.y; t.c100 = (float)p10.x; t.c110 = (float)p10.y;
    t.c001 = (float)p01.x; t.c011 = (float)p01.y; t.c101 = (float)p11.x; t.c111 = (float)p11.y;
  }
}

template <int VT, int AM>
__device__ __forceinline__ void tap_issue(const VolConsts& vc, f3 p, Tap& t)
{
  tap_coords(vc, p, t);
  tap_loads<VT, AM>(vc, t);
// ... 271 lines not shown
constexpr int kRunMax = 16;

struct ShadeReq {
  float px, py, pz;
  float s;
  float v;
  float tr;
  float a;
  int next;
};
static_assert(sizeof(ShadeReq) == kShadeReqBytes, "launch_plan.hpp restates the request's size");

__device__ __forceinline__ float bperm(int src_lane, float x)
{
  return __int_as_float(__builtin_amdgcn_ds_bpermute(src_lane << 2, __float_as_int(x)));
}
__device__ __forceinline__ int bperm_i(int src_lane, int x) { return __builtin_amdgcn_ds_bpermute(src_lane << 2, x); }

__device__ __forceinline__ unsigned int beam_index(const PoolDesc& Q, float px, float py, float pz)
{
  const int G = Q.order_grid;
  const int cu = min(max((int)fmaf(px, Q.order_u[0], fmaf(py, Q.order_u[1], fmaf(pz, Q.order_u[2], Q.order_u[3]))), 0), G - 1);
  const int cv = min(max((int)fmaf(px, Q.order_v[0], fmaf(py, Q.order_v[1], fmaf(pz, Q.order_v[2], Q.order_v[3]))), 0), G - 1);
  return ((unsigned int)(cu + 3 * cv) & 7u) * (unsigned int)(G * G / 8) + (unsigned int)(cv * (G / 8) + (cu >> 3));
}

__device__ __forceinline__ void setup_consts(const RayMarchParams& P, VolConsts& vc, MarchConsts& mc)
{
  vc.data = P.vol.data;
  vc.nx1 = P.vol.nx - 1; vc.ny1 = P.vol.ny - 1; vc.nz1 = P.vol.nz - 1;
  vc.macro_y = P.vol.macro_elems * (unsigned int)P.vol.macros_x;
  vc.macro_z = (unsigned long long)P.vol.macro_elems * (unsigned long long)P.vol.macros_x * (unsigned long long)P.vol.macros_y;
  vc.cs = ld3(P.coord_scale); vc.cb = ld3(P.coord_bias);
  vc.vscale = P.vol.value_scale; vc.vmin = P.vol.value_min_clamp;
  vc.majorant = P.majorant;
  vc.occupancy = P.occupancy;
  vc.occupancy_fine = P.occupancy_fine;
  vc.mcx1 = (P.vol.nx + 15) / 16 - 1; vc.mcy1 = (P.vol.ny + 15) / 16 - 1; vc.mcz1 = (P.vol.nz + 15) / 16 - 1;
  mc.inv_scale = ld3(P.inv_scale); mc.wto_p = ld3(P.wto_p); mc.otw_it = ld3(P.otw_it); mc.light = ld3(P.light);
  mc.gstep = ld3(P.grad_step);
  mc.ginv = mk3(1.f / mc.gstep.x, 1.f / mc.gstep.y, 1.f / mc.gstep.z);
  mc.step = P.step; mc.base = P.base; mc.shadow_stride = P.shadow_stride;
}

template <int VT, int AM>
__device__ __forceinline__ size_t stage_tables(const RayMarchParams& P, unsigned char* base, VolConsts& vc)
{
  vc.tab_x = vc.tab_y = vc.tab_z = nullptr;
  vc.tab_z64 = nullptr;
  if (AM == 3) return 0;
  const int na = Vox<VT>::kTransposed ? P.vol.ny : P.vol.nx, nb = Vox<VT>::kTransposed ? P.vol.nx : P.vol.ny;
  const unsigned int* __restrict__ gab = P.vol.axis_ab;
  const unsigned long long* __restrict__ gz = P.vol.axis_z;
  const int ea = axis_a_entries(na), nab = ea + axis_b_entries(nb), ez = axis_z_entries(P.vol.nz);
  if (AM == 2) {
    unsigned long long* tz = reinterpret_cast<unsigned long long*>(base);
    unsigned int* tx = reinterpret_cast<unsigned int*>(tz + ez);
    for (int i = threadIdx.x; i < nab; i += kBlock) tx[i] = gab[i];
    for (int i = threadIdx.x; i < ez; i += kBlock) tz[i] = gz[i];
    vc.tab_x = tx + 1; vc.tab_y = tx + ea + 1; vc.tab_z64 = tz + 1;
    return (size_t)ez * sizeof(unsigned long long) + (size_t)nab * sizeof(unsigned int);
  }
  unsigned int* tx = reinterpret_cast<unsigned int*>(base);
  unsigned int* tz = tx + nab;
  const unsigned int mul = (AM == 0 || AM == 4) ? (unsigned int)sizeof(typename Vox<VT>::T) : 1u;
  for (int i = threadIdx.x; i < nab; i += kBlock) tx[i] = gab[i] * mul;
  for (int i = threadIdx.x; i < ez; i += kBlock) tz[i] = (unsigned int)gz[i] * mul;
  vc.tab_x = tx + 1; vc.tab_y = tx + ea + 1; vc.tab_z = tz + 1;
  return (size_t)(nab + ez) * sizeof(unsigned int);
}
__device__ __forceinline__ void stage_tf(const RayMarchParams& P, unsigned char* tf_base, bool with_color, TfConsts& tf)
{
  float4* lc = reinterpret_cast<float4*>(tf_base);
  float* la = reinterpret_cast<float*>(tf_base + (with_color ? (size_t)(P.n_color + 1) * sizeof(float4) : 0));
  if (with_color) {
    const float4* gc = reinterpret_cast<const float4*>(P.tf_color);
    for (int i = threadIdx.x; i <= P.n_color; i += kBlock) lc[i] = gc[min(i, P.n_color - 1)];
  }
  for (int i = threadIdx.x; i < P.n_alpha; i += kBlock) la[i] = P.tf_alpha[i];
  if (threadIdx.x == 0) la[P.n_alpha] = P.tf_alpha[P.n_alpha - 1];
  __syncthreads();
  tf.color = lc;
  tf.alpha = la;
  tf.nc1 = P.n_color - 1; tf.na1 = P.n_alpha - 1;
  tf.fnc1 = (float)tf.nc1; tf.fna1 = (float)tf.na1;
  tf.lower = P.tf_lower; tf.upper = P.tf_upper; tf.scale = P.tf_scale;
}

__device__ __forceinline__ void write_pixel(const RayMarchParams& P, unsigned int pixel_index, f3 o_c, float o_a, f3 o_g)
{
  float4 out = make_float4(o_c.x, o_c.y, o_c.z, o_a);
  float4* fb = reinterpret_cast<float4*>(P.rgba) + pixel_index;
  if (P.accumulate) {
    float4* ac = reinterpret_cast<float4*>(P.accum) + pixel_index;
    if (P.accum_half && (P.frame_index & 1) == 0) {
      float4* hp = reinterpret_cast<float4*>(P.accum_half) + pixel_index;
      if (P.frame_index == 2) {
        *hp = out;
      }
      else {
        float4 h = *hp;
        h.x += out.x; h.y += out.y; h.z += out.z; h.w += out.w;
        *hp = h;
      }
    }
    if (P.frame_index == 1) {
      *ac = out;
// ... 178 lines not shown
}

__device__ __forceinline__ bool assign_pixel_quad(const RayMarchParams& P, int lane, int wave, int& ix, int& iy)
{
  const int ray = lane >> 2;
  bool active;
  if (P.sparse_xy) {
    const unsigned long long i = (unsigned long long)blockIdx.x * (kBlock / 4) + (unsigned int)(threadIdx.x >> 2);
    active = (2ull * i) < *P.sparse_count;
    ix = active ? P.sparse_xy[2 * i] : 0;
    iy = active ? P.sparse_xy[2 * i + 1] : 0;
  }
  else {
    const unsigned int e = P.schedule[blockIdx.x];
    ix = (int)(e & 0xffffu) * 8 + (wave & 1) * 4 + (ray & 3);
    iy = (int)(e >> 16) * 8 + (wave >> 1) * 4 + (ray >> 2);
    active = ix < P.width && iy < P.height;
  }
  if (P.world > 1 && active) active = ((ix / P.tile_w + iy / P.tile_h) % P.world) == P.rank;
  return active;
}

template <bool FINE>
__device__ __forceinline__ void skip_interval_level(const VolConsts& vc, f3 oo, f3 od, float t0, float t1, int sub, bool live, float& t_first, float& t_last)
{
  float first = FLT_MAX, last = -FLT_MAX;
  if (live) {
    const float len = t1 - t0;
    const float ta = fmaf((float)sub * 0.25f, len, t0), tb = sub == 3 ? t1 : fmaf((float)(sub + 1) * 0.25f, len, t0);
    skip_walk<FINE>(vc, oo, od, ta, tb, first, last);
  }
  t_first = fminf(fminf(quad_bcast<0>(first), quad_bcast<1>(first)), fminf(quad_bcast<2>(first), quad_bcast<3>(first)));
  t_last = fmaxf(fmaxf(quad_bcast<0>(last), quad_bcast<1>(last)), fmaxf(quad_bcast<2>(last), quad_bcast<3>(last)));
}
__device__ __forceinline__ SkipSpan skip_interval(const VolConsts& vc, f3 oo, f3 od, float t0, float t1, int sub, bool live)
{
  SkipSpan sp = skipspan_none();
  sp.mask_lo = sp.mask_hi = ~0u;
  skip_interval_level<false>(vc, oo, od, t0, t1, sub, live, sp.first, sp.last);
  const float c0 = sp.first, c1 = sp.last;
  const bool walk = live && c0 <= c1;
  if (__ballot(walk) != 0ull) skip_interval_level<true>(vc, oo, od, c0, c1, sub, walk, sp.first, sp.last);
  return sp;
}

constexpr int kMarchWavesPerEu = 3;
struct LdsRegion { int bx0, by0, bz0, ebx, eby, ebz, nbr, ok; };
static_assert(sizeof(LdsRegion) == kLdsRegionBytes, "launch_plan.hpp restates the region descriptor's size");
constexpr int kDeepK = 6;
constexpr int kPinMaxAM = 1;
template <int VT, int SHADE, int AM, bool POOLED, bool SKIP, bool LDSB = false, bool DEEP = false, bool MAT = false, bool CLIP = false, bool CACHED = false>
__global__ __launch_bounds__(kBlock) __attribute__((amdgpu_waves_per_eu((SKIP && POOLED && (AM == 4 ? 0 : AM) <= kPinMaxAM) ? kMarchWavesPerEu : 1, kMarchWavesPerEu))) void raymarch_kernel(const RayMarchParams P)
{
  static_assert(march_variant_exists(SHADE, AM, POOLED, SKIP, LDSB, DEEP, MAT, CLIP, VT == VOX_F32, CACHED), "no such variant of the march (host/launch_plan.hpp)");
  using Cfg = QCfg<SHADE, POOLED>;
  constexpr int K = DEEP ? kDeepK : Cfg::K;
  constexpr int QCAP = Cfg::QCAP;
  extern __shared__ __attribute__((aligned(16))) unsigned char lds_raw[];
  const int lane = threadIdx.x & 63, wave = threadIdx.x >> 6;
  const int sub = lane & 3;
  const int qbase = lane & ~3;
  const bool owner = sub == 0;
  const SubMask subm = make_submask(sub);
  const unsigned long long t_start = P.trace ? __builtin_amdgcn_s_memrealtime() : 0ull;

  int ix, iy;
  const bool active = assign_pixel_quad(P, lane, wave, ix, iy);
  unsigned int n_rays = 0, n_samples = 0, n_shaded = 0, n_shadow = 0, n_skipped = 0, n_shadow_skipped = 0, n_outside_hits = 0;
  VolConsts vc;
  MarchConsts mc;
  setup_consts(P, vc, mc);

  ShadeReq* const queue = reinterpret_cast<ShadeReq*>(lds_raw) + (size_t)wave * (QCAP > 0 ? QCAP : 1);
  TfConsts tf;
  SkipSpan pro_span = skipspan_none();
  const float rsx = 1.f / (float)P.width, rsy = 1.f / (float)P.height;
  const float scx = ((float)ix + .5f) * rsx, scy = ((float)iy + .5f) * rsy;
  const int spp = POOLED ? min(P.spp, 1) : P.spp;
  __shared__ float jit_lds[kJitStaged][2][64];
  const bool jit_staged = P.jitter_mode == 1 && !P.sparse_xy;
  if (jit_staged) {
    const unsigned int e = P.schedule[blockIdx.x];
    const int xy = P.jitter_xy, h = xy >> 1;
    const int nk = min(spp, kJitStaged);
    for (int i = threadIdx.x; i < nk * 128; i += kBlock) {
      const int k = i >> 7, d = (i >> 6) & 1, p = i & 63;
      const int px = (int)(e & 0xffffu) * 8 + (p & 7) + d * h, py = (int)(e >> 16) * 8 + (p >> 3) + d * h;
      jit_lds[k][d][p] = P.jitter_noise[(size_t)jitter_slice(P, (POOLED ? P.spp_index : 0) + k) * xy * xy + (size_t)(py % xy) * xy + (px % xy)];
    }
    __syncthreads();
  }
  auto jitter = [&](int k, float& x0, float& x1) {
    if (jit_staged && k < kJitStaged) {
      const int ray = lane >> 2;
      const int p = ((wave >> 1) * 4 + (ray >> 2)) * 8 + (wave & 1) * 4 + (ray & 3);
      x0 = jit_lds[k][0][p];
      x1 = jit_lds[k][1][p];
    }
    else jitter_global(P, ix, iy, (POOLED ? P.spp_index : 0) + k, x0, x1);
  };
  bool staged;
  {
    bool need = active;
    if (P.spp == 1 && active) {
      float sx0 = scx, sy0 = scy;
      if (P.jitter_mode == 1) {
        float j0, j1;
// ... 1267 lines not shown
  const long long i = ((long long)blockIdx.x * kBlock + threadIdx.x) >> 2;
  const bool valid = i < n;
  const long long j = valid ? i : 0;
  const f3 o = mk3(org[3 * j], org[3 * j + 1], org[3 * j + 2]), d = mk3(dir[3 * j], dir[3 * j + 1], dir[3 * j + 2]);
  const f3 oo = to_object(mc, o), od = mk3(d.x * mc.inv_scale.x, d.y * mc.inv_scale.y, d.z * mc.inv_scale.z);
  float t0 = 0.f, t1 = FLT_MAX;
  const bool live = valid && box_test<true>(P, t0, t1, oo, od);
  const IsoResult ir = isosurface_ray<VT, AM, 2, SKIP, true>(P, vc, mc, o, d, t0, t1, live, subm);
  if (valid && sub == 0) {
    float* q = out + 8 * i;
    q[0] = ir.hit ? 1.f : 0.f; q[1] = ir.hit ? ir.iso : 0.f; q[2] = ir.hit ? ir.t : 0.f; q[3] = live ? (float)ir.steps : 0.f;
    q[4] = ir.hit ? ir.n_w.x : 0.f; q[5] = ir.hit ? ir.n_w.y : 0.f; q[6] = ir.hit ? ir.n_w.z : 0.f; q[7] = ir.hit ? ir.shadow : 0.f;
  }
}

typedef void (*IsosurfaceFloatsKernel)(const RayMarchParams, const float*, const float*, float*, long long);
struct IsosurfaceKernels { FrameKernel frame = nullptr; IsosurfaceFloatsKernel floats = nullptr; };
template <int VT, int AM, int SHADE>
inline FrameKernel isosurface_frame_kernel(bool skip, bool clipped)
{
  if (skip) return clipped ? isosurface_kernel<VT, AM, SHADE, true, true> : isosurface_kernel<VT, AM, SHADE, true, false>;
  return clipped ? isosurface_kernel<VT, AM, SHADE, false, true> : isosurface_kernel<VT, AM, SHADE, false, false>;
}
template <int VT, int AM>
inline IsosurfaceKernels isosurface_kernels_of(int shade, bool skip, bool clipped)
{
  IsosurfaceKernels k;
  switch (shade) {
  case 0: k.frame = isosurface_frame_kernel<VT, AM, 0>(skip, clipped); break;
  case 1: k.frame = isosurface_frame_kernel<VT, AM, 1>(skip, clipped); break;
  case 2: k.frame = isosurface_frame_kernel<VT, AM, 2>(skip, clipped); break;
  default: return k;
  }
  k.floats = skip ? isosurface_floats_kernel<VT, AM, true> : isosurface_floats_kernel<VT, AM, false>;
  return k;
}
template <int VT>
IsosurfaceKernels isosurface_kernels_of(int am, int shade, bool skip, bool clipped)
{
  if constexpr (kVoxelTypes[VT].layout == LAYOUT_GENERAL) {
    switch (am) {
    case 0: return isosurface_kernels_of<VT, 0>(shade, skip, clipped);
    case 1: return isosurface_kernels_of<VT, 1>(shade, skip, clipped);
    case 2: return isosurface_kernels_of<VT, 2>(shade, skip, clipped);
    case 3: return isosurface_kernels_of<VT, 3>(shade, skip, clipped);
    case 4:
      if constexpr (row_load_layout((int)sizeof(typename Vox<VT>::T), Vox<VT>::kQuad)) return isosurface_kernels_of<VT, 4>(shade, skip, clipped);
      else return IsosurfaceKernels();
    }
  }
  return IsosurfaceKernels();
}

template <int VT>
FrameKernels frame_kernels(const LaunchPlan& pl)
{
  const unsigned flags = (pl.skip ? kBitSkip : 0u) | (pl.pooled ? kBitPooled : 0u) | (pl.march.lds_staged ? kBitLdsStaged : 0u) | (pl.march.deep ? kBitDeep : 0u);
  const unsigned march_bits = flags | (pl.march.material ? kBitMaterial : 0u) | (pl.march.clipped ? kBitClipped : 0u) | (pl.cached && !pl.pooled ? kBitCached : 0u);
  const unsigned shade_bits = (flags & kBitSkip) | (pl.shade.material ? kBitMaterial : 0u) | (pl.shade.clipped ? kBitClipped : 0u) | (pl.cached ? kBitCached : 0u);
  FrameKernels k;
  if (pl.error) return k;
  switch (pl.shading) {
  case 0: k = variants_of<VT, 0>(pl.am, march_bits, shade_bits); break;
  case 1: k = variants_of<VT, 1>(pl.am, march_bits, shade_bits); break;
  case 2: k = variants_of<VT, 2>(pl.am, march_bits, shade_bits); break;
  }
  if (!pl.pooled) k.shade = nullptr;
  return k;
}

}
```

open-volume-renderer_amd/csrc/ovr_hip_kernels.h:

```cpp
#pragma once

#include <hip/hip_runtime.h>
#include <stdint.h>
#include <type_traits>

#include "host/launch_plan.hpp"

namespace ovrhip {

enum VoxelType : int { VOX_U8 = 0, VOX_I8 = 1, VOX_U16 = 2, VOX_I16 = 3, VOX_F32 = 4, VOX_F32_T = 5, VOX_F32_TT = 6, VOX_U16_T = 7, VOX_U16_TT = 8, VOX_F32_Q = 9,
                       VOX_U16_Q = 10, VOX_U8_Q = 11 };
enum VolumeLayout : int { LAYOUT_GENERAL = 0, LAYOUT_THIN = 1, LAYOUT_THIN_T = 2, LAYOUT_QUAD = 3 };
constexpr int kLayouts = 4;
#define OVR_VOXEL_TYPES(X) \
  X(VOX_U8, u8, VOX_U8, LAYOUT_GENERAL) \
  X(VOX_I8, i8, VOX_I8, LAYOUT_GENERAL) \
  X(VOX_U16, u16, VOX_U16, LAYOUT_GENERAL) \
  X(VOX_I16, i16, VOX_I16, LAYOUT_GENERAL) \
  X(VOX_F32, f32, VOX_F32, LAYOUT_GENERAL) \
  X(VOX_F32_T, f32t, VOX_F32, LAYOUT_THIN) \
  X(VOX_F32_TT, f32tt, VOX_F32, LAYOUT_THIN_T) \
  X(VOX_U16_T, u16t, VOX_U16, LAYOUT_THIN) \
  X(VOX_U16_TT, u16tt, VOX_U16, LAYOUT_THIN_T) \
  X(VOX_F32_Q, f32q, VOX_F32, LAYOUT_QUAD) \
  X(VOX_U16_Q, u16q, VOX_U16, LAYOUT_QUAD) \
  X(VOX_U8_Q, u8q, VOX_U8, LAYOUT_QUAD)
struct VoxelTypeInfo { int type; const char* name; int base; int layout; };
#define OVR_X(E, NAME, BASE, LAYOUT) { E, #NAME, BASE, LAYOUT },
constexpr VoxelTypeInfo kVoxelTypes[] = { OVR_VOXEL_TYPES(OVR_X) };
#undef OVR_X
constexpr int kVoxelTypeCount = (int)(sizeof(kVoxelTypes) / sizeof(kVoxelTypes[0]));
constexpr bool voxel_types_match_enum()
{
  for (int i = 0; i < kVoxelTypeCount; ++i)
    if (kVoxelTypes[i].type != i || kVoxelTypes[kVoxelTypes[i].base].layout != LAYOUT_GENERAL) return false;
  return true;
}
static_assert(kVoxelTypeCount == 12 && VOX_U8_Q == 11 && voxel_types_match_enum(), "the list restates the VoxelType enum: entry i is the type of value i");
template <bool GENERAL_ONLY = false, typename F>
inline bool dispatch_voxel_type(int voxel_type, F&& f)
{
  switch (voxel_type) {
#define OVR_X(E, NAME, BASE, LAYOUT) \
  case E: \
    if constexpr (!GENERAL_ONLY || LAYOUT == LAYOUT_GENERAL) { f(std::integral_constant<int, E>{}); return true; } \
    else return false;
    OVR_VOXEL_TYPES(OVR_X)
#undef OVR_X
  default: return false;
  }
}
template <typename F> inline bool dispatch_general_voxel_type(int voxel_type, F&& f) { return dispatch_voxel_type<true>(voxel_type, f); }
constexpr int replica_voxel_type(int base_voxel_type, int layout)
{
  for (const VoxelTypeInfo& t : kVoxelTypes)
    if (t.base == base_voxel_type && t.layout == layout) return t.type;
  return -1;
}
constexpr int kBlockCounters = 8;

struct VolumeDesc {
  const void* data;
  int type;
  int nx, ny, nz;
  int macros_x, macros_y, macros_z;
  unsigned int macro_elems;
  unsigned long long bytes;
  float value_scale;
  float value_min_clamp;
  const unsigned int* axis_ab;
  const unsigned long long* axis_z;
};
__host__ __device__ constexpr int axis_a_entries(int na) { return na + 1; }
__host__ __device__ constexpr int axis_b_entries(int nb) { return nb + 2; }
__host__ __device__ constexpr int axis_z_entries(int nz) { return nz + 2; }

struct float3_ { float x, y, z; };

constexpr int kPoolSubs = 4;
constexpr int kPoolCtrlWords = 32 * (kPoolSubs + 2);
struct PoolDesc {
  struct ShadeReq* reqs;
  unsigned int capacity;
  unsigned int sub_capacity;
  unsigned int* ctrl;
  int* chunk_next;
  unsigned int* chunk_n;
  int* tile_first;
  unsigned int* tile_count;
  float4* pix_state;
  unsigned int* shade_counters;
  unsigned int* order;
  unsigned int* order_key;
  unsigned int* order_ws;
  int order_grid;
  float order_u[4], order_v[4];
};
constexpr int kOrderMaxGrid = 128;
constexpr int kOrderMaxKeys = kOrderMaxGrid * kOrderMaxGrid;
constexpr unsigned int kOrderNoKey = 0xffffffffu;
constexpr int kOrderLists = 8;
constexpr int kOrderHist = 0;
constexpr int kOrderFill = kOrderMaxKeys;
constexpr int kOrderListStart = 2 * kOrderMaxKeys;
constexpr int kOrderTickets = kOrderListStart + 32;
constexpr int kOrderWsWords = kOrderTickets + kOrderLists * 32;

struct RayMarchParams {
  float* rgba;
  float* grad;
  float* accum;
  float* accum_half;
  int width, height;
  int frame_index;
  int accumulate;
  int spp;
  int spp_index;
  int row_loads;
  float* spp_sum_rgba;
  float* spp_sum_grad;
  float3_ cam_pos, cam_dir, cam_hor, cam_ver;
  float3_ inv_scale, wto_p, otw_it;
  float wtc_it[9];
  float3_ light;
  float3_ coord_scale, coord_bias, grad_step;
  float step, base;
// ... 1 lines not shown
  float long_ray_steps;
  float tf_lower, tf_upper, tf_scale;
  const float* tf_color;
  const float* tf_alpha;
  int n_color, n_alpha;
  int shading;
  int rank, world, tile_w, tile_h;
  const unsigned int* schedule;
  unsigned int n_schedule;
  unsigned int n_blocks_owned;
  const int32_t* sparse_xy;
  const unsigned long long* sparse_count;
  unsigned long long sparse_hint_pixels;
  int jitter_mode, jitter_xy;
  const float* jitter_noise;
  int lds_staging;
  int shade_blocks;
  unsigned int lds_brick_offset;
  unsigned long long* counters;
  unsigned long long* publish;
  unsigned int* reduce_done;
  int zero_first;
  unsigned int* conv_asked;
  const float* majorant;
  const unsigned char* occupancy;
  const unsigned char* occupancy_fine;
  unsigned long long* trace;
  unsigned int* block_counters;
  PoolDesc pool;
  VolumeDesc vol;
  float mat_ka, mat_kd, mat_ks, mat_shininess, light_i2;
  float3_ clip_lo, clip_hi;
  int clip_on;
  const float* shadow_lattice;
  int shadow_n1[3];
  int projection;
  const float* mc_ranges;
  int iso_n;
  float iso_values[4];
};

struct ShadowBuildArgs {
  float* out;
  const float* pos;
  float* pos_out;
  long long n;
  int nx, ny, nz;
  float sc[3], origin[3];
  unsigned long long* iterations;
};
hipError_t launch_shadow_cache(const RayMarchParams& p, const ShadowBuildArgs& a, hipStream_t stream);
hipError_t launch_shadow_lookup(const RayMarchParams& p, const float* pos, float* out, int64_t n, hipStream_t stream);

LaunchPlan plan_raymarch(const RayMarchParams& p);
hipError_t launch_raymarch(const RayMarchParams& p, const LaunchPlan& plan, hipStream_t stream, const hipEvent_t* ev);
size_t pool_shade_blocks();
size_t raymarch_lds_bytes(int n_color, int n_alpha);
int volume_addressing_mode(const VolumeDesc& vd, int n_color, int n_alpha);
size_t raymarch_grid_blocks(const RayMarchParams& p);
size_t schedule_workspace_elems(unsigned int n);
hipError_t launch_schedule(const RayMarchParams& p, const unsigned int* src, unsigned int n, unsigned int* dst, unsigned int* workspace, int exact, unsigned int* info,
                           hipStream_t stream);
hipError_t launch_clear_blocks(const RayMarchParams& p, const unsigned int* blocks, unsigned int n, int clear_accum, hipStream_t stream);

hipError_t launch_project_floats(const RayMarchParams& p, const float* org, const float* dir, float* out, int64_t n, int mode, int range_skipping, hipStream_t stream);

hipError_t launch_isosurface_floats(const RayMarchParams& p, const float* org, const float* dir, float* out, int64_t n, int range_skipping, hipStream_t stream);

struct ConvergenceParams {
  const float* accum;
  const float* accum_half;
  const float* grad;
  float* grad_keep;
  int width, height, frame_index;
  int rank, world, tile_w, tile_h;
  int blocks_x;
  int adaptive;
  float threshold;
  const unsigned int* sorted;
  unsigned int n_work;
  const unsigned int* active;
  unsigned int n_active;
  unsigned int* active_out;
  unsigned int* retired_out;
  unsigned int* counts;
  float* block_error;
  int* block_frames;
  unsigned int* words;
  unsigned int sub_capacity;
  unsigned int* publish;
};
hipError_t launch_convergence(const ConvergenceParams& c, hipStream_t stream);
hipError_t launch_resolve_blocks(const RayMarchParams& p, const unsigned int* retired, unsigned int n, const int* block_frames, const float* grad_keep, int blocks_x,
                                 hipStream_t stream);

constexpr int kReconMaxLevels = 20;
struct ReconParams {
  float* rgba;
  float* grad;
  const float* count;
  const float* accum;
  const float* grad_sum;
  int width, height;
  int levels;
  int top;
  int level_w[kReconMaxLevels], level_h[kReconMaxLevels];
  unsigned int level_offset[kReconMaxLevels];
  float4* pyramid;
// ... 65 lines not shown
```

open-volume-renderer_amd/csrc/ovr_hip_kernels.hip:

```cpp
#include "ovr_hip_device.h"
#include "ovr_hip_update.h"

namespace ovrhip {
static_assert(kPoolSubs <= 64 && (kPoolSubs & (kPoolSubs - 1)) == 0, "reduce_counters_kernel reduces the sub-pool counters with one wave");
__global__ __launch_bounds__(kBlock) void composite_kernel(const RayMarchParams P)
{
  const int lane = threadIdx.x & 63, wave = threadIdx.x >> 6;
  int ix, iy;
  const bool active = assign_pixel_quad(P, lane, wave, ix, iy) && (lane & 3) == 0;
  const PoolDesc& Q = P.pool;
  if (Q.ctrl[1] != 0u) return;
  const unsigned int tile = blockIdx.x * kWaves + wave;
  const unsigned int pixel_index = (unsigned int)ix + (unsigned int)iy * (unsigned int)P.width;
  float alpha = 0.f;
  unsigned int first = 0;
  int pend = 0;
  if (active) {
    const float4 st = Q.pix_state[pixel_index];
    alpha = st.x; first = __float_as_uint(st.y); pend = __float_as_int(st.z);
  }
  f3 color = mk3(0, 0, 0), gradient = mk3(0, 0, 0);
  const unsigned int total = Q.tile_count[tile];
  auto load_chunk = [&](int c, unsigned int n) {
    ShadeReq r;
// ... 790 lines not shown
      Q.order_ws[kOrderTickets + 32 * threadIdx.x] = 0u;
    }
    if (threadIdx.x == 255) Q.order_ws[kOrderListStart + kOrderLists] = s_wave[0] + s_wave[1] + s_wave[2] + s_wave[3];
  }
  const unsigned int rps = Q.sub_capacity / (unsigned int)kRun, slots = rps * (unsigned int)kPoolSubs;
  unsigned int key[kOrderSlots], gid[kOrderSlots];
#pragma unroll
  for (int k = 0; k < kOrderSlots; ++k) {
    gid[k] = (blockIdx.x * (unsigned int)kOrderSlots + (unsigned int)k) * 256u + threadIdx.x;
    key[k] = kOrderNoKey;
    if (gid[k] < slots) {
      const unsigned int sub = gid[k] / rps, run = gid[k] - sub * rps;
      if (run < min(Q.ctrl[32u * (sub + 1u)], Q.sub_capacity) / (unsigned int)kRun) key[k] = Q.order_key[gid[k]];
    }
  }
#pragma unroll
  for (int k = 0; k < kOrderSlots; ++k) {
    if (key[k] >= (unsigned int)n) continue;
    const unsigned int pos = s_off[key[k]] + atomicAdd(&Q.order_ws[kOrderFill + key[k]], 1u);
    if (pos < slots) Q.order[pos] = gid[k];
  }
}

static hipError_t launch_shade_order(const RayMarchParams& q, hipStream_t stream)
{
  const unsigned int slots = q.pool.capacity / (unsigned int)kRun;
  const dim3 grid((slots + 256u * kOrderSlots - 1u) / (256u * kOrderSlots));
  if (grid.x == 0) return hipSuccess;
  const size_t lds = (size_t)q.pool.order_grid * q.pool.order_grid * sizeof(unsigned int);
  if (lds >= 48 * 1024) {
    hipError_t e = hipFuncSetAttribute(reinterpret_cast<const void*>(shade_order_kernel), hipFuncAttributeMaxDynamicSharedMemorySize, (int)lds);
    if (e != hipSuccess) return e;
  }
  hipLaunchKernelGGL(shade_order_kernel, grid, dim3(256), lds, stream, q);
  return hipGetLastError();
}

constexpr int kReduceBlocks = 64;
static hipError_t launch_reduce_counters(const unsigned int* partials, int n_blocks, const unsigned int* shade_partials, int n_shade_blocks,
                                         unsigned long long* counters, unsigned int* pool_ctrl, unsigned long long* publish, unsigned int* done, hipStream_t stream,
                                         unsigned int* conv_asked)
{
  hipLaunchKernelGGL(reduce_counters_kernel, dim3(kReduceBlocks), dim3(256), 0, stream, partials, n_blocks, shade_partials, n_shade_blocks, counters, pool_ctrl,
                     done ? publish : nullptr, done, conv_asked);
  return hipGetLastError();
}

#define OVR_X(E, NAME, BASE, LAYOUT) extern template FrameKernels frame_kernels<E>(const LaunchPlan&);
OVR_VOXEL_TYPES(OVR_X)
#undef OVR_X

size_t pool_shade_blocks() { return kShadeBlocks; }

LaunchPlan plan_raymarch(const RayMarchParams& p)
{
  static const int deep = getenv("OVR_HIP_DEEP") ? atoi(getenv("OVR_HIP_DEEP")) : -1;
  static const int shade_blocks = getenv("OVR_HIP_SHADE_BLOCKS") ? atoi(getenv("OVR_HIP_SHADE_BLOCKS")) : 0;
  LaunchOverrides o;
  if (const char* a = getenv("OVR_HIP_ADDRESSING")) o.addressing = atoi(a);
  o.deep = deep;
  o.shade_blocks = shade_blocks;
  LaunchFacts f;
  f.elem_bytes = (int)voxel_size(p.vol.type);
  f.quad = p.vol.type >= 0 && p.vol.type < kVoxelTypeCount && kVoxelTypes[p.vol.type].layout == LAYOUT_QUAD;
  f.f32_general = p.vol.type == VOX_F32;
  f.nx = p.vol.nx; f.ny = p.vol.ny; f.nz = p.vol.nz;
  f.stored_bytes = p.vol.bytes;
  f.tables = p.vol.axis_ab && p.vol.axis_z;
  f.n_color = p.n_color; f.n_alpha = p.n_alpha; f.shading = p.shading;
  f.pool = p.pool.reqs != nullptr; f.skipping = p.majorant != nullptr; f.sparse = p.sparse_xy != nullptr;
  f.sparse_hint_pixels = p.sparse_hint_pixels;
  f.world = p.world;
  f.n_blocks_owned = p.n_blocks_owned; f.n_schedule = p.n_schedule; f.schedule = p.schedule != nullptr;
  f.clip_on = p.clip_on != 0; f.lds_staging = p.lds_staging != 0;
  f.row_loads = p.row_loads; f.shade_blocks = p.shade_blocks;
  f.reference_material = reference_material(p); f.shade_order = p.pool.order != nullptr;
  f.shadow_cache = p.shadow_lattice != nullptr;
  f.projection = p.projection; f.ranges = p.mc_ranges != nullptr;
  f.isosurfaces = p.iso_n;
  return plan_launch(f, o);
}

static hipError_t launch_variant(FrameKernel kern, dim3 grid, size_t lds, hipStream_t stream, const RayMarchParams& prm)
{
  if (lds > 64 * 1024)
    if (hipError_t e = hipFuncSetAttribute(reinterpret_cast<const void*>(kern), hipFuncAttributeMaxDynamicSharedMemorySize, (int)lds)) return e;
  if (grid.x > 0) hipLaunchKernelGGL(kern, grid, dim3(kBlock), lds, stream, prm);
  return hipSuccess;
}

static hipError_t launch_sequence(const RayMarchParams& p, const LaunchPlan& plan, const FrameKernels& k, hipStream_t stream, const hipEvent_t* ev)
{
  const dim3 grid((unsigned)raymarch_grid_blocks(p));
  hipError_t e;
  if (!plan.pooled) {
    RayMarchParams q = p;
    if (plan.march.lds_staged) q.lds_brick_offset = plan.lds_brick_offset;
    if ((e = launch_variant(k.march, grid, plan.march_lds_bytes, stream, q)) != hipSuccess) return e;
    if ((e = hipGetLastError()) != hipSuccess) return e;
    if (ev && ev[1] && ev[2]) { (void)hipEventRecord(ev[1], stream); (void)hipEventRecord(ev[2], stream); }
    if (p.block_counters && p.counters) {
      if (!p.publish || p.zero_first)
        if ((e = hipMemsetAsync(p.counters, 0, 8 * sizeof(unsigned long long), stream)) != hipSuccess) return e;
      if ((e = launch_reduce_counters(p.block_counters, (int)grid.x, nullptr, 0, p.counters, nullptr, p.publish, p.reduce_done, stream, p.conv_asked)) != hipSuccess) return e;
    }
    return hipGetLastError();
  }
  const bool self_cleaning = p.publish && p.block_counters && p.counters && !p.zero_first;
  if (!self_cleaning) {
    if ((e = hipMemsetAsync(p.pool.ctrl, 0, (size_t)kPoolCtrlWords * sizeof(unsigned int), stream)) != hipSuccess) return e;
    if (p.block_counters && p.counters)
      if ((e = hipMemsetAsync(p.counters, 0, 8 * sizeof(unsigned long long), stream)) != hipSuccess) return e;
  }
  RayMarchParams q = p;
  if (!plan.shade_order) q.pool.order = nullptr;
  for (int g = 0; g < p.spp; ++g) {
    q.spp_index = g;
    if (g > 0 && (e = hipMemsetAsync(p.pool.ctrl, 0, (size_t)32 * (kPoolSubs + 1) * sizeof(unsigned int), stream)) != hipSuccess) return e;
    if ((e = launch_variant(k.march, grid, plan.march_lds_bytes, stream, q)) != hipSuccess) return e;
    if ((e = hipGetLastError()) != hipSuccess) return e;
    if (ev && ev[1] && g == p.spp - 1) (void)hipEventRecord(ev[1], stream);
    if (q.pool.order && (e = launch_shade_order(q, stream)) != hipSuccess) return e;
    if ((e = launch_variant(k.shade, dim3((unsigned)plan.shade_grid_blocks), plan.shade_lds_bytes, stream, q)) != hipSuccess) return e;
    if ((e = hipGetLastError()) != hipSuccess) return e;
    if (ev && ev[2] && g == p.spp - 1) (void)hipEventRecord(ev[2], stream);
    if (grid.x > 0 && (e = launch_composite(q, grid, stream)) != hipSuccess) return e;
    if (p.block_counters && p.counters)
      if ((e = launch_reduce_counters(p.block_counters, (int)grid.x, (const unsigned int*)p.pool.shade_counters, plan.shade_grid_blocks, p.counters, p.pool.ctrl,
                                      g == p.spp - 1 ? p.publish : nullptr, p.reduce_done, stream, p.conv_asked)) != hipSuccess) return e;
  }
  return hipGetLastError();
}

#define OVR_X(E, NAME, BASE, LAYOUT) extern template ProjectKernels project_kernels_of<E>(int, int, bool, bool);
OVR_VOXEL_TYPES(OVR_X)
#undef OVR_X
static ProjectKernels project_kernels(const RayMarchParams& p, const LaunchPlan& plan)
{
  ProjectKernels k;
  if (!plan.error) dispatch_voxel_type(p.vol.type, [&](auto vt) { k = project_kernels_of<decltype(vt)::value>(plan.am, plan.project.mode, plan.project.skip, plan.project.clipped); });
  return k;
}

#define OVR_X(E, NAME, BASE, LAYOUT) extern template IsosurfaceKernels isosurface_kernels_of<E>(int, int, bool, bool);
OVR_VOXEL_TYPES(OVR_X)
#undef OVR_X
static IsosurfaceKernels isosurface_kernels(const RayMarchParams& p, const LaunchPlan& plan)
{
  IsosurfaceKernels k;
  if (!plan.error && plan.isosurface.on)
    dispatch_voxel_type<true>(p.vol.type, [&](auto vt) { k = isosurface_kernels_of<decltype(vt)::value>(plan.am, plan.shading, plan.isosurface.skip, plan.isosurface.clipped); });
  return k;
}

hipError_t launch_raymarch(const RayMarchParams& p, const LaunchPlan& plan, hipStream_t stream, const hipEvent_t* ev)
{
  if (ev) (void)hipEventRecord(ev[0], stream);
  FrameKernels k;
  if (plan.isosurface.on) k.march = isosurface_kernels(p, plan).frame;
  else if (plan.project.mode != 0) k.march = project_kernels(p, plan).frame;
  else dispatch_voxel_type(p.vol.type, [&](auto vt) { k = frame_kernels<decltype(vt)::value>(plan); });
  const hipError_t e = k.march && (k.shade || !plan.pooled) ? launch_sequence(p, plan, k, stream, ev) : hipErrorInvalidValue;
  if (ev) (void)hipEventRecord(ev[3], stream);
  return e;
}

template <typename TI_, int VT_> struct ValueTypeOf { typedef TI_ TI; typedef typename Vox<VT_>::T TO; static constexpr int VT = VT_; };
template <typename F>
static bool dispatch_value_type(int ovr_value_type, F&& f)
{
  switch (ovr_value_type) {
  case 100: f(ValueTypeOf<unsigned char, VOX_U8>{}); return true;
  case 101: f(ValueTypeOf<signed char, VOX_I8>{}); return true;
  case 200: f(ValueTypeOf<unsigned short, VOX_U16>{}); return true;
  case 201: f(ValueTypeOf<short, VOX_I16>{}); return true;
  case 300: f(ValueTypeOf<unsigned int, VOX_F32>{}); return true;
  case 301: f(ValueTypeOf<int, VOX_F32>{}); return true;
  case 400: f(ValueTypeOf<float, VOX_F32>{}); return true;
  case 500: f(ValueTypeOf<double, VOX_F32>{}); return true;
  default: return false;
  }
}
int device_voxel_type(int t)
{
  int vt = -1;
  dispatch_value_type(t, [&](auto v) { vt = decltype(v)::VT; });
  return vt;
}
size_t voxel_size(int vt)
{
  size_t bytes = 4;
  dispatch_voxel_type(vt, [&](auto t) { bytes = sizeof(typename Vox<decltype(t)::value>::T); });
  return bytes;
}

template <typename TI, typename TO> struct Conv { static __device__ __forceinline__ TO cv(TI v) { return (TO)v; } };
template <> struct Conv<unsigned int, float> {
  static __device__ __forceinline__ float cv(unsigned int v) { return (float)v / (float)0xffffffffu; }
};
template <> struct Conv<int, float> {
  static __device__ __forceinline__ float cv(int v) { const float n = (float)v / (float)0x7fffffff; return n < -1.f ? -1.f : n; }
};

template <typename TI> struct SrcLinear {
  typedef TI value_type;
  static constexpr bool kLinear = true;
  const TI* p; int nx, ny, z0;
  __device__ __forceinline__ TI get(size_t x, size_t y, unsigned z) const { return p[x + (size_t)nx * (y + (size_t)ny * (size_t)(z - (unsigned)z0))]; }
};
template <int VTB> struct SrcBricked {
  typedef typename Vox<VTB>::T value_type;
  static constexpr bool kLinear = false;
  static constexpr bool kBox = false;
  const value_type* p; unsigned int macro_y; unsigned long long macro_z;
  __device__ __forceinline__ value_type get(size_t x, size_t y, unsigned z) const
// ... 115 lines not shown
  typedef typename V::T TO;
  typedef typename V::Q Q;
  const unsigned my = blockIdx.x, layer = ((unsigned)z0 >> V::lz) + blockIdx.y;
  const unsigned long long slab = S::slab(my, layer, macro_y, macro_z);
  const unsigned total = (unsigned)macros_x * S::CELLS;
  for (unsigned g = threadIdx.x; g < total; g += 256u) {
    const unsigned mx = g / S::CELLS, i = g - mx * S::CELLS;
    const unsigned j = i & (S::CB - 1u), brick = i / S::CB;
    const int u = (int)(mx * 32u + ((brick & (M::bx_ - 1u)) << V::lx) + (j & ((1u << V::lx) - 1u)));
    const int v = (int)(my * 32u + ((brick / M::bx_) << V::ly) + ((j >> V::lx) & ((1u << V::ly) - 1u)));
    const unsigned z = (layer << V::lz) + (j >> (V::lx + V::ly));
    Q* const cell = reinterpret_cast<Q*>(dst + slab + (unsigned long long)mx * M::MV + (unsigned long long)i * 4u);
    if (u > nx || v > ny || z >= (unsigned)nz) {
      if (z >= (unsigned)z0) { Q zero; zero.x = zero.y = zero.z = zero.w = (TO)0; *cell = zero; }
      continue;
    }
    if (z < (unsigned)z0 || z >= (unsigned)(z0 + nz_chunk)) continue;
    const int x = max(u - 1, 0), y = max(v - 1, 0);
    const int x1 = min(u, nx - 1), y1 = min(v, ny - 1);
    Q q;
    q.x = Conv<TI, TO>::cv(src.get((size_t)x, (size_t)y, z)); q.y = Conv<TI, TO>::cv(src.get((size_t)x1, (size_t)y, z));
    q.z = Conv<TI, TO>::cv(src.get((size_t)x, (size_t)y1, z)); q.w = Conv<TI, TO>::cv(src.get((size_t)x1, (size_t)y1, z));
    *cell = q;
  }
}
template <typename SRC, int VT>
static hipError_t relayout_quad_s(const SRC& src, void* dst, const VolumeDesc& vd, int z0, int nzc, hipStream_t stream)
{
  if (nzc <= 0) return hipSuccess;
  const unsigned last = z0 + nzc >= vd.nz ? (unsigned)vd.macros_z * (32u >> Vox<VT>::lz) - 1u : (unsigned)(z0 + nzc - 1) >> Vox<VT>::lz;
  dim3 grid((unsigned)vd.macros_y, last - ((unsigned)z0 >> Vox<VT>::lz) + 1u);
  hipLaunchKernelGGL((relayout_quad_kernel<SRC, VT>), grid, dim3(256), 0, stream, src, (typename Vox<VT>::T*)dst, vd.nx, vd.ny, vd.macros_x, macro_stride_y(vd),
                     macro_stride_z(vd), z0, nzc, vd.nz);
  return hipGetLastError();
}

template <typename SRC, typename TO, int VT>
static hipError_t relayout_s(const SRC& src, void* dst, const VolumeDesc& vd, int z0, int nzc, hipStream_t stream)
{
  if (nzc <= 0) return hipSuccess;
  const unsigned last = z0 + nzc >= vd.nz ? (unsigned)vd.macros_z * (32u >> Vox<VT>::bz) - 1u : (unsigned)(z0 + nzc - 1) >> Vox<VT>::bz;
  const unsigned layers = last - ((unsigned)z0 >> Vox<VT>::bz) + 1u;
  dim3 grid((unsigned)vd.macros_y, layers);
  hipLaunchKernelGGL((relayout_kernel<SRC, TO, VT>), grid, dim3(256), 0, stream, src, (TO*)dst, vd.nx, vd.ny, vd.macros_x, macro_stride_y(vd), macro_stride_z(vd), z0, nzc,
                     vd.nz);
  return hipGetLastError();
}

template <int VT>
static void volume_layout_t(int nx, int ny, int nz, VolumeDesc& vd)
{
  typedef BrickMap<VT> M;
  const int na = Vox<VT>::kTransposed ? ny : nx, nb = Vox<VT>::kTransposed ? nx : ny;
  vd.macros_x = (na + 1 + (int)M::MCX - 1) / (int)M::MCX;
  vd.macros_y = ((Vox<VT>::kQuad ? nb + 1 : nb) + 31) / 32;
  vd.macros_z = (nz + 31) / 32;
  vd.macro_elems = M::MV;
  vd.bytes = (unsigned long long)vd.macros_x * vd.macros_y * vd.macros_z * M::MV * sizeof(typename Vox<VT>::T);
}
bool volume_layout(int voxel_type, int nx, int ny, int nz, VolumeDesc& vd)
{
  return dispatch_voxel_type(voxel_type, [&](auto vt) {
    vd.type = voxel_type;
    vd.nx = nx; vd.ny = ny; vd.nz = nz;
    volume_layout_t<decltype(vt)::value>(nx, ny, nz, vd);
  });
}

hipError_t launch_relayout(const void* src, int vt, void* dst, const VolumeDesc& vd, int z0, int nzc, hipStream_t stream)
{
  hipError_t e = hipErrorInvalidValue;
  dispatch_value_type(vt, [&](auto v) {
    typedef decltype(v) V;
    typedef SrcLinear<typename V::TI> Src;
    if (vd.type == V::VT) e = relayout_s<Src, typename V::TO, V::VT>(Src{ (const typename V::TI*)src, vd.nx, vd.ny, z0 }, dst, vd, z0, nzc, stream);
  });
  return e;
}

template <int VTB>
static hipError_t rebrick_b(const VolumeDesc& g, void* dst, const VolumeDesc& vd, int z0, int nzc, hipStream_t stream)
{
  typedef typename Vox<VTB>::T T;
  typedef SrcBricked<VTB> Src;
  constexpr int T1 = replica_voxel_type(VTB, LAYOUT_THIN), T2 = replica_voxel_type(VTB, LAYOUT_THIN_T), TQ = replica_voxel_type(VTB, LAYOUT_QUAD);
  if constexpr (TQ >= 0) { if (vd.type == TQ) return relayout_quad_s<Src, TQ>(src_bricked<VTB>(g), dst, vd, z0, nzc, stream); }
  if constexpr (T1 >= 0) { if (vd.type == T1) return relayout_s<Src, T, T1>(src_bricked<VTB>(g), dst, vd, z0, nzc, stream); }
  if constexpr (T2 >= 0) { if (vd.type == T2) return relayout_s<Src, T, T2>(src_bricked<VTB>(g), dst, vd, z0, nzc, stream); }
  return hipErrorInvalidValue;
}
hipError_t launch_rebrick(const VolumeDesc& general, void* dst, const VolumeDesc& vd, hipStream_t stream)
{
  for (int z0 = 0; z0 < vd.nz; z0 += 32768) {
    const int nzc = std::min(32768, vd.nz - z0);
    hipError_t e = hipErrorInvalidValue;
    dispatch_general_voxel_type(general.type, [&](auto vtb) { e = rebrick_b<decltype(vtb)::value>(general, dst, vd, z0, nzc, stream); });
    if (e != hipSuccess) return e;
  }
  return hipSuccess;
}

template <typename TI> struct SrcBox {
  typedef TI value_type;
  static constexpr bool kBox = true;
  const TI* p; int x0, y0, z0, ex, ey;
  __device__ __forceinline__ TI get(size_t x, size_t y, unsigned z) const { return p[(x - (size_t)x0) + (size_t)ex * ((y - (size_t)y0) + (size_t)ey * (size_t)(z - (unsigned)z0))]; }
};
struct UpdateRows { int alo, ahi, blo, bhi, zlo, zhi; int brick_lo, brick_hi, macro_lo, macros, row_lo, layer_lo; };

template <typename SRC, typename TO, int VT>
__global__ __launch_bounds__(256) void update_rows_kernel(const SRC src, TO* __restrict__ dst, int nx, int ny, unsigned int macro_y, unsigned long long macro_z, const UpdateRows u)
{
  typedef typename SRC::value_type TI;
  typedef RowSweep<VT> S;
  typedef Vox<VT> V;
  constexpr bool TR = V::kTransposed;
  constexpr unsigned SX = S::SX;
  const int na = TR ? ny : nx;
  const unsigned my = (unsigned)u.row_lo + blockIdx.x, layer = (unsigned)u.layer_lo + blockIdx.y;
  const unsigned long long slab = S::slab(my, layer, macro_y, macro_z);
  const unsigned total = (unsigned)u.macros * S::ROWS;
  for (unsigned g = threadIdx.x; g < total; g += 256u) {
    const typename S::Row r = S::decode(g, (unsigned)u.macro_lo, my, layer);
    const int b = (int)r.b, z = (int)r.z;
    const int br = (int)r.br;
    if (b < u.blo || b >= u.bhi || z < u.zlo || z >= u.zhi || br < u.brick_lo || br > u.brick_hi) continue;
    RowOut<TO, SX>* const row = S::row(dst, slab, r);
    const int v0 = br * V::cx - 1;
    RowOut<TO, SX> out;
    if constexpr (SRC::kBox) {
      static_assert(!TR, "the caller's array goes into the general layout");
      if (v0 >= u.alo && v0 + (int)SX <= u.ahi) {
        const RowIn<TI, SX> w = *reinterpret_cast<const RowIn<TI, SX>*>(&src.p[((size_t)v0 - (size_t)src.x0) + (size_t)src.ex * (((size_t)b - (size_t)src.y0) + (size_t)src.ey * (size_t)(z - src.z0))]);
#pragma unroll
        for (unsigned k = 0; k < SX; ++k) out.v[k] = Conv<TI, TO>::cv(w.v[k]);
      }
      else {
        out = *row;
#pragma unroll
        for (unsigned k = 0; k < SX; ++k) {
          const int as = min(max(v0 + (int)k, 0), na - 1);
          if (as >= u.alo && as < u.ahi) out.v[k] = Conv<TI, TO>::cv(src.get((size_t)as, (size_t)b, (unsigned)z));
        }
      }
    }
    else {
#pragma unroll
      for (unsigned k = 0; k < SX; ++k) {
        const size_t as = (size_t)min(max(v0 + (int)k, 0), na - 1);
        out.v[k] = Conv<TI, TO>::cv(TR ? src.get((size_t)b, as, (unsigned)z) : src.get(as, (size_t)b, (unsigned)z));
      }
    }
    *row = out;
  }
}

struct UpdateCells { int u_lo, u_hi, v_lo, v_hi, zlo, zhi; int macro_lo, macros, row_lo, layer_lo; };
template <typename SRC, int VT>
__global__ __launch_bounds__(256) void update_quad_kernel(const SRC src, typename Vox<VT>::T* __restrict__ dst, int nx, int ny, unsigned int macro_y, unsigned long long macro_z,
                                                         const UpdateCells c)
{
  typedef typename SRC::value_type TI;
  typedef QuadSweep<VT> S;
  typedef BrickMap<VT> M;
  typedef Vox<VT> V;
  typedef typename V::T TO;
  typedef typename V::Q Q;
  const unsigned my = (unsigned)c.row_lo + blockIdx.x, layer = (unsigned)c.layer_lo + blockIdx.y;
  const unsigned long long slab = S::slab(my, layer, macro_y, macro_z);
  const unsigned total = (unsigned)c.macros * S::CELLS;
  for (unsigned g = threadIdx.x; g < total; g += 256u) {
    const unsigned ml = g / S::CELLS, i = g - ml * S::CELLS, mx = (unsigned)c.macro_lo + ml;
    const unsigned j = i & (S::CB - 1u), brick = i / S::CB;
    const int u = (int)(mx * 32u + ((brick & (M::bx_ - 1u)) << V::lx) + (j & ((1u << V::lx) - 1u)));
    const int v = (int)(my * 32u + ((brick / M::bx_) << V::ly) + ((j >> V::lx) & ((1u << V::ly) - 1u)));
    const int z = (int)((layer << V::lz) + (j >> (V::lx + V::ly)));
    if (u < c.u_lo || u > c.u_hi || v < c.v_lo || v > c.v_hi || z < c.zlo || z >= c.zhi) continue;
    Q* const cell = reinterpret_cast<Q*>(dst + slab + (unsigned long long)mx * M::MV + (unsigned long long)i * 4u);
    const int x = max(u - 1, 0), y = max(v - 1, 0);
    const int x1 = min(u, nx - 1), y1 = min(v, ny - 1);
    Q q;
    q.x = Conv<TI, TO>::cv(src.get((size_t)x, (size_t)y, (unsigned)z)); q.y = Conv<TI, TO>::cv(src.get((size_t)x1, (size_t)y, (unsigned)z));
    q.z = Conv<TI, TO>::cv(src.get((size_t)x, (size_t)y1, (unsigned)z)); q.w = Conv<TI, TO>::cv(src.get((size_t)x1, (size_t)y1, (unsigned)z));
    *cell = q;
  }
}

template <int VT> static update::Geometry update_geometry()
{
  typedef Vox<VT> V;
  update::Geometry g{ V::cx, V::mbx, V::by, V::bz, V::kTransposed, V::kQuad, 0, 0, 0 };
  if constexpr (V::kQuad) { g.lx = V::lx; g.ly = V::ly; g.lz = V::lz; }
  return g;
}
constexpr int kUpdateLayers = 32768;

template <typename SRC, typename TO, int VT>
static hipError_t update_rows_s(const SRC& src, void* dst, const VolumeDesc& vd, const update::Box& box, hipStream_t stream)
{
  const int dims[3] = { vd.nx, vd.ny, vd.nz };
  const update::BrickRange r = update::brick_range(update_geometry<VT>(), dims, vd.macros_x, box);
  constexpr int ia = Vox<VT>::kTransposed ? 1 : 0, ib = Vox<VT>::kTransposed ? 0 : 1;
  for (int l0 = r.layer_lo; l0 <= r.layer_hi; l0 += kUpdateLayers) {
    const UpdateRows u{ box.lo[ia], box.hi[ia], box.lo[ib], box.hi[ib], box.lo[2], box.hi[2], r.brick_lo, r.brick_hi, r.macro_lo, r.macro_hi - r.macro_lo + 1, r.row_lo, l0 };
    const dim3 grid((unsigned)(r.row_hi - r.row_lo + 1), (unsigned)(std::min(r.layer_hi, l0 + kUpdateLayers - 1) - l0 + 1));
    hipLaunchKernelGGL((update_rows_kernel<SRC, TO, VT>), grid, dim3(256), 0, stream, src, (TO*)dst, vd.nx, vd.ny, macro_stride_y(vd), macro_stride_z(vd), u);
    if (hipError_t e = hipGetLastError()) return e;
  }
  return hipSuccess;
}
template <typename SRC, int VT>
static hipError_t update_quad_s(const SRC& src, void* dst, const VolumeDesc& vd, const update::Box& box, hipStream_t stream)
{
  const update::QuadRange r = update::quad_range(update_geometry<VT>(), box);
  for (int l0 = r.layer_lo; l0 <= r.layer_hi; l0 += kUpdateLayers) {
    const UpdateCells c{ r.u_lo, r.u_hi, r.v_lo, r.v_hi, box.lo[2], box.hi[2], r.macro_lo, r.macro_hi - r.macro_lo + 1, r.row_lo, l0 };
    const dim3 grid((unsigned)(r.row_hi - r.row_lo + 1), (unsigned)(std::min(r.layer_hi, l0 + kUpdateLayers - 1) - l0 + 1));
    hipLaunchKernelGGL((update_quad_kernel<SRC, VT>), grid, dim3(256), 0, stream, src, (typename Vox<VT>::T*)dst, vd.nx, vd.ny, macro_stride_y(vd), macro_stride_z(vd), c);
    if (hipError_t e = hipGetLastError()) return e;
  }
  return hipSuccess;
}
hipError_t launch_update_general(const void* src, int vt, void* dst, const VolumeDesc& vd, const update::Box& box, hipStream_t stream)
{
  hipError_t e = hipErrorInvalidValue;
  dispatch_value_type(vt, [&](auto v) {
    typedef decltype(v) V;
    typedef SrcBox<typename V::TI> Src;
    if (vd.type == V::VT)
      e = update_rows_s<Src, typename V::TO, V::VT>(Src{ (const typename V::TI*)src, box.lo[0], box.lo[1], box.lo[2], box.hi[0] - box.lo[0], box.hi[1] - box.lo[1] }, dst, vd, box, stream);
  });
  return e;
}
template <int VTB>
static hipError_t update_replica_b(const VolumeDesc& g, void* dst, const VolumeDesc& vd, const update::Box& box, hipStream_t stream)
{
  typedef typename Vox<VTB>::T T;
  typedef SrcBricked<VTB> Src;
  constexpr int T1 = replica_voxel_type(VTB, LAYOUT_THIN), T2 = replica_voxel_type(VTB, LAYOUT_THIN_T), TQ = replica_voxel_type(VTB, LAYOUT_QUAD);
  if constexpr (TQ >= 0) { if (vd.type == TQ) return update_quad_s<Src, TQ>(src_bricked<VTB>(g), dst, vd, box, stream); }
  if constexpr (T1 >= 0) { if (vd.type == T1) return update_rows_s<Src, T, T1>(src_bricked<VTB>(g), dst, vd, box, stream); }
  if constexpr (T2 >= 0) { if (vd.type == T2) return update_rows_s<Src, T, T2>(src_bricked<VTB>(g), dst, vd, box, stream); }
  return hipErrorInvalidValue;
}
hipError_t launch_update_replica(const VolumeDesc& general, void* dst, const VolumeDesc& vd, const update::Box& box, hipStream_t stream)
{
  hipError_t e = hipErrorInvalidValue;
  dispatch_general_voxel_type(general.type, [&](auto vtb) { e = update_replica_b<decltype(vtb)::value>(general, dst, vd, box, stream); });
  return e;
}

template <int VT>
__global__ __launch_bounds__(256) void axis_tables_kernel(VolumeDesc vd, unsigned int* __restrict__ ab, unsigned long long* __restrict__ tz)
{
  typedef BrickMap<VT> M;
  const int na = Vox<VT>::kTransposed ? vd.ny : vd.nx, nb = Vox<VT>::kTransposed ? vd.nx : vd.ny;
  const unsigned int macro_y = macro_stride_y(vd);
  const unsigned long long macro_z = macro_stride_z(vd);
  const int i = (int)(blockIdx.x * 256u + threadIdx.x);
  if (i < axis_a_entries(na)) ab[i] = M::X((unsigned)i);
  if (i < axis_b_entries(nb)) ab[axis_a_entries(na) + i] = M::Y(Vox<VT>::kQuad ? (unsigned)min(i, nb) : (unsigned)min(max(i - 1, 0), nb - 1), macro_y);
  if (i < axis_z_entries(vd.nz)) {
    const unsigned z = (unsigned)min(max(i - 1, 0), vd.nz - 1);
    tz[i] = (unsigned long long)M::Zlo(z) + (unsigned long long)(z >> 5) * macro_z;
  }
}
size_t axis_table_bytes(const VolumeDesc& vd)
{
  return (size_t)axis_z_entries(vd.nz) * sizeof(unsigned long long) + (size_t)(vd.nx + vd.ny + 3) * sizeof(unsigned int);
}
template <int VT>
static hipError_t axis_tables_t(const VolumeDesc& vd, unsigned int* ab, unsigned long long* tz, hipStream_t stream)
{
  const int n = std::max(std::max(vd.nx, vd.ny), vd.nz) + 2;
  hipLaunchKernelGGL(axis_tables_kernel<VT>, dim3((unsigned)((n + 255) / 256)), dim3(256), 0, stream, vd, ab, tz);
  return hipGetLastError();
}
hipError_t launch_axis_tables(VolumeDesc& vd, void* d_tables, hipStream_t stream)
{
  unsigned long long* tz = static_cast<unsigned long long*>(d_tables);
  unsigned int* ab = reinterpret_cast<unsigned int*>(tz + axis_z_entries(vd.nz));
  vd.axis_z = tz;
  vd.axis_ab = ab;
  hipError_t e = hipErrorInvalidValue;
  dispatch_voxel_type(vd.type, [&](auto vt) { e = axis_tables_t<decltype(vt)::value>(vd, ab, tz, stream); });
  return e;
}

template <int VT>
__device__ __forceinline__ float2 macrocell_cell_range(const void* __restrict__ vol, const VolumeDesc& vd, int cx, int cy, int cz, int lane)
{
  typedef BrickMap<VT> M;
  typedef Vox<VT> V;
  typedef typename V::T T;
  constexpr unsigned SX = M::SX, HY = 1u << V::by, HZ = 1u << V::bz;
  constexpr int W = 16;
  constexpr unsigned AY = (W + 2 + 2 * (HY - 1) + HY - 1) / HY, AZ = (W + 2 + 2 * (HZ - 1) + HZ - 1) / HZ;
  const int bx = max(cx * W - 1, 0), by = max(cy * W - 1, 0), bz = max(cz * W - 1, 0);
  const int ex = min(bx + W + 1, vd.nx), ey = min(by + W + 1, vd.ny), ez = min(bz + W + 1, vd.nz);
  const unsigned macro_y = macro_stride_y(vd);
  const unsigned long long macro_z = macro_stride_z(vd);
  const T* base = static_cast<const T*>(vol);
  const unsigned b0 = M::div_cx((unsigned)bx + 1u), nbx = M::div_cx((unsigned)ex) - b0 + 1u;
  const unsigned ya = (unsigned)by & ~(HY - 1u), za = (unsigned)bz & ~(HZ - 1u);
  float lo = INFINITY, hi = -INFINITY;
  for (unsigned t = (unsigned)lane; t < AY * AZ * HY * HZ; t += 64u) {
    const unsigned q = t / (HY * HZ);
    const unsigned y = ya + (q % AY) * HY + (t & (HY - 1u)), z = za + (q / AY) * HZ + ((t / HY) & (HZ - 1u));
    if ((int)y < by || (int)y >= ey || (int)z < bz || (int)z >= ez) continue;
    const unsigned long long row = (unsigned long long)M::Y(y, macro_y) + M::Zlo(z) + (unsigned long long)(z >> 5) * macro_z;
    for (unsigned qx = 0; qx < nbx; ++qx) {
      const unsigned br = b0 + qx;
      const unsigned m = M::div_mbx(br), bm = br - m * V::mbx;
      const RowOut<T, SX> w = *reinterpret_cast<const RowOut<T, SX>*>(base + (row + (bm * M::BV + m * M::MV)));
      const int v0 = (int)(br * V::cx) - 1;
#pragma unroll
      for (unsigned k = 0; k < SX; ++k) {
        float f = (float)w.v[k];
        if (VT == VOX_U8) f = f / 255.f;
        if (VT == VOX_I8) { f = f / 127.f; f = f < -1.f ? -1.f : f; }
        const bool in = v0 + (int)k >= bx && v0 + (int)k < ex;
        lo = in ? fminf(lo, f) : lo;
// ... 565 lines not shown
```

Baseline: 94080.

## Add compact f32 brick replica for march pass on large sparse-ray volumes

Adds a new compact f32 volume replica layout without the x-apron. It uses 4-wide bricks that each fill one 128-byte line, built in the background like other replicas. When the general layout is chosen, the volume exceeds 1 GiB and rays are sparse relative to volume size, the pooled march kernel reads from the compact replica. Shading still uses the general layout. This aims to cut memory traffic and cache footprint in the march, at the cost of extra device memory, build work, and added plan and update complexity.

```diff
diff --git a/open-volume-renderer_amd/csrc/host/compact_layout.hpp b/open-volume-renderer_amd/csrc/host/compact_layout.hpp
--- /dev/null
+++ b/open-volume-renderer_amd/csrc/host/compact_layout.hpp
@@ -0,0 +1,37 @@
+#pragma once
+
+#if defined(__HIPCC__)
+#define OVR_COMPACT_HD __host__ __device__ __forceinline__
+#else
+#define OVR_COMPACT_HD inline
+#endif
+
+namespace ovrhip {
+namespace compact {
+
+constexpr int kCx = 4, kMbx = 8, kBy = 2, kBz = 1;
+
+struct Map {
+  static constexpr unsigned SX = kCx;
+  static constexpr unsigned BV = SX << (kBy + kBz);
+  static constexpr unsigned sby = kMbx * BV, sbz = (32u >> kBy) * kMbx * BV;
+  static constexpr unsigned MV = (32u >> kBz) * sbz;
+  static constexpr unsigned MCX = kCx * kMbx;
+  static OVR_COMPACT_HD unsigned div_cx(unsigned x) { return x >> 2; }
+  static OVR_COMPACT_HD unsigned div_mbx(unsigned b) { return b >> 3; }
+  static OVR_COMPACT_HD unsigned X(unsigned u) { return (u & 3u) + ((u >> 2) & 7u) * BV + (u >> 5) * MV; }
+  static OVR_COMPACT_HD unsigned Y(unsigned y, unsigned macro_y_stride) { return (y & 3u) * SX + ((y >> 2) & 7u) * sby + (y >> 5) * macro_y_stride; }
+  static OVR_COMPACT_HD unsigned Zlo(unsigned z) { return ((z & 1u) << kBy) * SX + ((z >> 1) & 15u) * sbz; }
+};
+static_assert(Map::BV * 4 == 128 && Map::MV == 32u * 32u * 32u && Map::MCX == 32, "a brick is one 128-byte line, a macro block 32^3 cells");
+
+constexpr int macros_x(int nx) { return (nx + 2 + 31) / 32; }
+constexpr int macros_y(int ny) { return (ny + 31) / 32; }
+constexpr int macros_z(int nz) { return (nz + 31) / 32; }
+constexpr unsigned long long elements(int nx, int ny, int nz)
+{
+  return (unsigned long long)macros_x(nx) * (unsigned long long)macros_y(ny) * (unsigned long long)macros_z(nz) * Map::MV;
+}
+
+}
+}
diff --git a/open-volume-renderer_amd/csrc/host/frame.cpp b/open-volume-renderer_amd/csrc/host/frame.cpp
--- a/open-volume-renderer_amd/csrc/host/frame.cpp
+++ b/open-volume-renderer_amd/csrc/host/frame.cpp
@@ -232,6 +232,7 @@
     (void)hipGetLastError();
   }
   choice = r->tune.before_frame(choice, tune_l, tune_p, building);
+  r->layout_asked = choice;
   choice = resolve_layout(r, choice, may_wait, st);
   const float vs = P.vol.value_scale, vm = P.vol.value_min_clamp;
   P.vol = r->vd_replica[choice];
@@ -248,6 +249,7 @@
   P.vol.value_scale = vs;
   P.vol.value_min_clamp = vm;
   r->stats.layout = LAYOUT_GENERAL;
+  r->layout_asked = LAYOUT_GENERAL;
   r->tune.frame = -1;
 }
 
@@ -620,8 +622,19 @@
   const bool phases = r->phase_timing.load();
   hipEvent_t evs[4] = { r->ev[0], phases ? r->ev[1] : nullptr, phases ? r->ev[2] : nullptr, r->ev[3] };
   r->frame_phase_timed = phases;
-  r->plan = plan_raymarch(r->P);
-  HIP_TRY(launch_raymarch(r->P, r->plan, st, evs));
+  const VolumeDesc* compact = nullptr;
+  if (r->layout_asked == LAYOUT_GENERAL && r->replica_state[LAYOUT_COMPACT].load(std::memory_order_acquire) != 0) {
+    r->plan = plan_raymarch(r->P, &r->vd_replica[LAYOUT_COMPACT], r->march_compact);
+    if (r->plan.march.compact) {
+      if (r->replica_state[LAYOUT_COMPACT] == 1) (void)start_replica_build(r, LAYOUT_COMPACT, nullptr);
+      int state = r->replica_state[LAYOUT_COMPACT].load(std::memory_order_acquire);
+      if (state == 2 && hipEventQuery(r->build_ev[LAYOUT_COMPACT]) == hipSuccess) { r->replica_state[LAYOUT_COMPACT] = 3; state = 3; }
+      (void)hipGetLastError();
+      if (state == 3) compact = &r->vd_replica[LAYOUT_COMPACT];
+    }
+  }
+  if (!compact) r->plan = plan_raymarch(r->P);
+  HIP_TRY(launch_raymarch(r->P, r->plan, st, evs, compact));
   r->frame_words_dirty = false;
   if (r->conv.frame) {
     ConvergenceParams c{};
diff --git a/open-volume-renderer_amd/csrc/host/launch_plan.hpp b/open-volume-renderer_amd/csrc/host/launch_plan.hpp
--- a/open-volume-renderer_amd/csrc/host/launch_plan.hpp
+++ b/open-volume-renderer_amd/csrc/host/launch_plan.hpp
@@ -22,8 +22,9 @@
 
 constexpr bool row_load_layout(int elem_bytes, bool quad) { return elem_bytes <= 2 && !quad; }
 constexpr bool march_variant_exists(int shade, int am, bool pooled, bool skip, bool lds_staged, bool deep, bool material, bool clipped, bool f32_general,
-                                    bool cached = false)
-{
+                                    bool cached = false, bool compact = false)
+{
+  if (compact) return shade >= 1 && shade <= 2 && am >= 0 && am <= 2 && pooled && !skip && !lds_staged && !deep && !material && !clipped && !cached && !f32_general;
   if (cached && !(shade == 1 && material && !pooled)) return false;
   if (shade < 0 || shade > 2 || am < 0 || am > 4 || (f32_general && am == 4)) return false;
   if (pooled && shade == 0) return false;
@@ -75,6 +76,18 @@
   const size_t tables = axis_table_bytes(nx, ny, nz, am);
   const size_t fixed = tf_lds_bytes(n_color, n_alpha) + (size_t)kWaves * request_queue_entries(1, false) * kShadeReqBytes + 1024;
   return ((am == 2 && tables > 64 * 1024) || tables + 16 + fixed > 160 * 1024) ? 3 : am;
+}
+
+constexpr unsigned long long kCompactMinBytes = 1ull << 30;
+constexpr bool compact_march_pays(int elem_bytes, bool f32_general, unsigned long long general_bytes, int choice)
+{
+  return f32_general && elem_bytes == 4 && choice != 0 && (choice > 0 || general_bytes > kCompactMinBytes);
+}
+inline bool compact_rays_sparse(unsigned long long rays, int nx, int ny, int nz, int choice)
+{
+  if (choice >= 0) return choice > 0;
+  const long double r = (long double)rays, v = (long double)nx * (long double)ny * (long double)nz;
+  return rays > 0 && r * r * r <= v * v;
 }
 
 struct LaunchFacts {
@@ -97,14 +110,15 @@
   int projection = 0;
   bool ranges = false;
   int isosurfaces = 0;
+  unsigned long long compact_bytes = 0;
 };
-struct LaunchOverrides { int addressing = -1, deep = -1, shade_blocks = 0; };
+struct LaunchOverrides { int addressing = -1, deep = -1, shade_blocks = 0, compact = -1; };
 
 struct LaunchPlan {
   int shading = 0;
   int am = 0;
   bool pooled = false, skip = false;
-  struct March { bool lds_staged = false, deep = false, material = false, clipped = false; } march;
+  struct March { bool lds_staged = false, deep = false, material = false, clipped = false, compact = false; int compact_am = 0; } march;
   struct Shade { bool material = false, clipped = false; } shade;
   bool shade_order = false;
   bool cached = false;
@@ -197,6 +211,17 @@
   pl.march_lds_bytes = queues + tables + (size_t)f.n_alpha * 4 + 64;
   pl.march.clipped = f.clip_on;
   pl.march.deep = !f.skipping && (am <= 1 || am == 4) && !f.clip_on && deep_rounds_pay(f, o);
+  const unsigned long long rays = f.sparse ? f.sparse_hint_pixels : 64ull * f.n_schedule * (unsigned long long)std::max(f.world, 1);
+  if (f.compact_bytes > 0 && compact_march_pays(f.elem_bytes, f.f32_general, f.stored_bytes, o.compact) && compact_rays_sparse(rays, f.nx, f.ny, f.nz, o.compact) &&
+      !pl.skip && !pl.march.clipped && !pl.march.deep) {
+    int cam = addressing_mode(f.compact_bytes, f.elem_bytes, f.nx, f.ny, f.nz, f.n_color, f.n_alpha);
+    if (o.addressing >= 0) cam = std::min(std::max(cam, o.addressing), 3);
+    if (march_variant_exists(sh, cam, true, false, false, false, false, false, false, false, true)) {
+      pl.march.compact = true;
+      pl.march.compact_am = cam;
+      pl.march_lds_bytes = queues + align16(axis_table_bytes(f.nx, f.ny, f.nz, cam) + 4) + (size_t)f.n_alpha * 4 + 64;
+    }
+  }
   pl.shade.clipped = sh == 2 && f.clip_on;
   pl.shade.material = pl.shade.clipped || !f.reference_material || pl.cached;
   pl.shade_order = sh == 2 && f.shade_order;
diff --git a/open-volume-renderer_amd/csrc/host/state.hpp b/open-volume-renderer_amd/csrc/host/state.hpp
--- a/open-volume-renderer_amd/csrc/host/state.hpp
+++ b/open-volume-renderer_amd/csrc/host/state.hpp
@@ -191,13 +191,13 @@
   void* d_volume = nullptr;
   std::atomic<size_t> volume_bytes{ 0 };
   ovrhip::VolumeDesc vd{};
-  void* d_replica[ovrhip::kLayouts] = {};
-  void* d_axis[ovrhip::kLayouts] = {};
-  ovrhip::VolumeDesc vd_replica[ovrhip::kLayouts] = {};
-  std::atomic<int> replica_state[ovrhip::kLayouts] = {};
-  std::thread builder[ovrhip::kLayouts];
+  void* d_replica[ovrhip::kReplicaSlots] = {};
+  void* d_axis[ovrhip::kReplicaSlots] = {};
+  ovrhip::VolumeDesc vd_replica[ovrhip::kReplicaSlots] = {};
+  std::atomic<int> replica_state[ovrhip::kReplicaSlots] = {};
+  std::thread builder[ovrhip::kReplicaSlots];
   hipStream_t build_stream = nullptr;
-  hipEvent_t build_ev[ovrhip::kLayouts] = {};
+  hipEvent_t build_ev[ovrhip::kReplicaSlots] = {};
   int value_type = 0;
   float origin[3] = { 0, 0, 0 }, spacing[3] = { 1, 1, 1 };
   bool have_volume = false;
@@ -212,6 +212,8 @@
   ovrhip::policy::AutoPipeline auto_pipe;
   ovrhip::policy::Skip skip;
   bool shade_order_on = true;
+  int layout_asked = 0;
+  int march_compact = -1;
   float shade_beam = 32.f;
 
   float* d_mc_minmax = nullptr;
diff --git a/open-volume-renderer_amd/csrc/host/update_extent.hpp b/open-volume-renderer_amd/csrc/host/update_extent.hpp
--- a/open-volume-renderer_amd/csrc/host/update_extent.hpp
+++ b/open-volume-renderer_amd/csrc/host/update_extent.hpp
@@ -8,7 +8,7 @@
 
 struct Box { int lo[3], hi[3]; };
 
-struct Geometry { int cx, mbx, by, bz; bool transposed, quad; int lx, ly, lz; };
+struct Geometry { int cx, mbx, by, bz; bool transposed, quad; int lx, ly, lz; int apron = 1; };
 
 enum { kOk = 0, kNull = 1, kMemKind = 2, kType = 3, kExtent = 4, kOutside = 5 };
 inline int check_arguments(const void* data, const int32_t* lower, const int32_t* extent, int mem_kind, int value_type, int resident_type, const int dims[3])
@@ -41,10 +41,10 @@
   int layer_lo, layer_hi;
 };
 
-inline void pair_axis_bricks(int cx, int na, int bricks_total, int a, int b, int& lo, int& hi)
+inline void pair_axis_bricks(int cx, int na, int bricks_total, int a, int b, int& lo, int& hi, int apron = 1)
 {
   const int p_lo = a == 0 ? 0 : a + 1;
-  lo = p_lo == 0 ? 0 : (p_lo - 1) / cx;
+  lo = p_lo == 0 ? 0 : (p_lo - apron) / cx;
   hi = b == na ? bricks_total - 1 : std::min(b / cx, bricks_total - 1);
 }
 
@@ -52,7 +52,7 @@
 {
   const int ia = g.transposed ? 1 : 0, ib = g.transposed ? 0 : 1;
   BrickRange r;
-  pair_axis_bricks(g.cx, dims[ia], macros_a * g.mbx, box.lo[ia], box.hi[ia], r.brick_lo, r.brick_hi);
+  pair_axis_bricks(g.cx, dims[ia], macros_a * g.mbx, box.lo[ia], box.hi[ia], r.brick_lo, r.brick_hi, g.apron);
   r.macro_lo = r.brick_lo / g.mbx; r.macro_hi = r.brick_hi / g.mbx;
   r.row_lo = box.lo[ib] >> 5; r.row_hi = (box.hi[ib] - 1) >> 5;
   r.layer_lo = box.lo[2] >> g.bz; r.layer_hi = (box.hi[2] - 1) >> g.bz;
diff --git a/open-volume-renderer_amd/csrc/host/volume.cpp b/open-volume-renderer_amd/csrc/host/volume.cpp
--- a/open-volume-renderer_amd/csrc/host/volume.cpp
+++ b/open-volume-renderer_amd/csrc/host/volume.cpp
@@ -235,7 +235,7 @@
 
 void join_builders(ovr_hip_renderer* r)
 {
-  for (int k = 0; k < kLayouts; ++k)
+  for (int k = 0; k < kReplicaSlots; ++k)
     if (r->builder[k].joinable()) r->builder[k].join();
 }
 
@@ -314,7 +314,7 @@
 int poll_replica_builds(ovr_hip_renderer* r)
 {
   int building = 0;
-  for (int k = 1; k < kLayouts; ++k) {
+  for (int k = 1; k < kReplicaSlots; ++k) {
     int state = r->replica_state[k].load(std::memory_order_acquire);
     if (state == 2 && hipEventQuery(r->build_ev[k]) == hipSuccess) { r->replica_state[k] = 3; state = 3; }
     if (state == 2 || state == 4) building++;
@@ -350,6 +350,14 @@
       if (plan(LAYOUT_QUAD, tq) && layout_offsets_fit(tq) && (r->layouts.current == 2 || (double)tq.bytes + planned <= 0.4 * (double)free_b)) {
         r->vd_replica[LAYOUT_QUAD] = tq;
         r->replica_state[LAYOUT_QUAD] = 1;
+        planned += (double)tq.bytes;
+      }
+    }
+    if (r->layouts.current != 0 && replica_voxel_type(vt, LAYOUT_COMPACT) >= 0 && compact_march_pays((int)voxel_size(vt), vt == VOX_F32, vd.bytes, r->march_compact)) {
+      VolumeDesc tc;
+      if (plan(LAYOUT_COMPACT, tc) && layout_offsets_fit(tc) && (r->layouts.current == 2 || (double)tc.bytes + planned <= 0.4 * (double)free_b)) {
+        r->vd_replica[LAYOUT_COMPACT] = tc;
+        r->replica_state[LAYOUT_COMPACT] = 1;
       }
     }
   }
@@ -437,7 +445,7 @@
   auto t_seg = std::chrono::high_resolution_clock::now();
   join_builders(r);
   HIP_TRY(hipStreamSynchronize(r->build_stream));
-  for (int k = 0; k < kLayouts; ++k) {
+  for (int k = 0; k < kReplicaSlots; ++k) {
     if (r->d_replica[k]) HIP_TRY(hipFree(r->d_replica[k]));
     r->d_replica[k] = nullptr;
     if (r->d_axis[k]) HIP_TRY(hipFree(r->d_axis[k]));
@@ -465,17 +473,17 @@
   t_seg = std::chrono::high_resolution_clock::now();
   r->vd = vd;
   if (r->layouts.current == 2) {
-    for (int k = 1; k < kLayouts; ++k) {
+    for (int k = 1; k < kReplicaSlots; ++k) {
       if (r->replica_state[k] != 1) continue;
       std::string err;
       (void)start_replica_build(r, k, &err, false);
       if (r->replica_state[k] != 2) {
-        for (int j = 1; j < kLayouts; ++j) drop_replica(r, j);
+        for (int j = 1; j < kReplicaSlots; ++j) drop_replica(r, j);
         return fail(OVR_HIP_EDEVICE, std::string("[hip] volume replicas requested (layouts mode 2) but their allocation failed: ") + err);
       }
     }
     HIP_TRY(hipStreamSynchronize(r->build_stream));
-    for (int k = 1; k < kLayouts; ++k)
+    for (int k = 1; k < kReplicaSlots; ++k)
       if (r->replica_state[k] == 2) r->replica_state[k] = 3;
   }
   r->value_type = value_type;
@@ -516,7 +524,7 @@
   for (int k = 0; k < 3; ++k) { box.lo[k] = lower[k]; box.hi[k] = lower[k] + extent[k]; }
 
   join_builders(r);
-  for (int k = 1; k < kLayouts; ++k)
+  for (int k = 1; k < kReplicaSlots; ++k)
     if (r->replica_state[k].load(std::memory_order_acquire) == 2) HIP_TRY(hipStreamWaitEvent(st, r->build_ev[k], 0));
 
   const size_t in_es = value_type_size(value_type);
@@ -562,7 +570,7 @@
     const auto t_seg = std::chrono::high_resolution_clock::now();
     VolumeDesc g = r->vd_replica[LAYOUT_GENERAL];
     g.data = r->d_volume;
-    for (int k = 1; k < kLayouts; ++k) {
+    for (int k = 1; k < kReplicaSlots; ++k) {
       const int state = r->replica_state[k].load(std::memory_order_acquire);
       if (state == 2 || state == 3) HIP_TRY(launch_update_replica(g, r->d_replica[k], r->vd_replica[k], box, st));
     }
diff --git a/open-volume-renderer_amd/csrc/ovr_hip_api.cpp b/open-volume-renderer_amd/csrc/ovr_hip_api.cpp
--- a/open-volume-renderer_amd/csrc/ovr_hip_api.cpp
+++ b/open-volume-renderer_amd/csrc/ovr_hip_api.cpp
@@ -47,7 +47,7 @@
       if (hipDeviceGetStreamPriorityRange(&lo, &hi) != hipSuccess) { (void)hipGetLastError(); lo = hi = 0; }
       HIP_TRY(hipStreamCreateWithPriority(&r->build_stream, hipStreamNonBlocking, hi));
     }
-    for (int k = 0; k < kLayouts; ++k) HIP_TRY(hipEventCreateWithFlags(&r->build_ev[k], hipEventDisableTiming));
+    for (int k = 0; k < kReplicaSlots; ++k) HIP_TRY(hipEventCreateWithFlags(&r->build_ev[k], hipEventDisableTiming));
     HIP_TRY(hipMalloc((void**)&r->d_counters, kFrameWordsBytes));
     HIP_TRY(hipMemset(r->d_counters, 0, kFrameWordsBytes));
     HIP_TRY(hipMalloc((void**)&r->d_sparse_count, sizeof(unsigned long long)));
@@ -70,6 +70,7 @@
   if (const char* f = getenv("OVR_HIP_SKIP_ADAPTIVE")) r->skip.adaptive = atoi(f) != 0;
   if (const char* f = getenv("OVR_HIP_TUNE")) r->tune.on = atoi(f) != 0;
   if (const char* f = getenv("OVR_HIP_SHADE_ORDER")) r->shade_order_on = atoi(f) != 0;
+  if (const char* f = getenv("OVR_HIP_MARCH_COMPACT")) r->march_compact = atoi(f) != 0 ? 1 : 0;
   if (const char* f = getenv("OVR_HIP_ROW_LOADS")) r->P.row_loads = atoi(f) != 0 ? 2 : 1;
   if (const char* f = getenv("OVR_HIP_SHADE_BEAM")) r->shade_beam = std::max(1.f, (float)atof(f));
   *out = r;
@@ -86,7 +87,7 @@
   (void)hipDeviceSynchronize();
   group_release(r);
   (void)free_framebuffers(r);
-  for (int k = 0; k < kLayouts; ++k) {
+  for (int k = 0; k < kReplicaSlots; ++k) {
     if (r->d_replica[k]) (void)hipFree(r->d_replica[k]);
     if (r->d_axis[k]) (void)hipFree(r->d_axis[k]);
   }
@@ -122,7 +123,7 @@
   for (int i = 0; i < 2; ++i)
     if (r->own_stream[i]) (void)hipStreamDestroy(r->own_stream[i]);
   if (r->build_stream) (void)hipStreamDestroy(r->build_stream);
-  for (int k = 0; k < kLayouts; ++k)
+  for (int k = 0; k < kReplicaSlots; ++k)
     if (r->build_ev[k]) (void)hipEventDestroy(r->build_ev[k]);
   delete r;
 }
diff --git a/open-volume-renderer_amd/csrc/ovr_hip_device.h b/open-volume-renderer_amd/csrc/ovr_hip_device.h
--- a/open-volume-renderer_amd/csrc/ovr_hip_device.h
+++ b/open-volume-renderer_amd/csrc/ovr_hip_device.h
@@ -1,5 +1,6 @@
 #pragma once
 #include "ovr_hip_kernels.h"
+#include "host/compact_layout.hpp"
 
 #include <float.h>
 #include <math.h>
@@ -183,6 +184,15 @@
   static constexpr bool kQuad = true;
 };
 
+template <> struct Vox<VOX_F32_C> {
+  typedef float T; typedef f32x2_u P;
+  static constexpr int cx = 4, mbx = 8, by = 2, bz = 1;
+  static_assert(cx == compact::kCx && mbx == compact::kMbx && by == compact::kBy && bz == compact::kBz, "host/compact_layout.hpp is this brick's map");
+  static constexpr bool kScale = false, kClamp = false;
+  static constexpr bool kTransposed = false;
+  static constexpr bool kQuad = false;
+};
+
 template <int VT> struct BrickMap {
   typedef Vox<VT> V;
   static constexpr unsigned SX = V::cx + 1;
@@ -226,6 +236,7 @@
     return (z & ((1u << V::lz) - 1u)) * (4u << (V::lx + V::ly)) + ((z >> V::lz) & ((32u >> V::lz) - 1u)) * (bx_ * by_ * BV);
   }
 };
+template <> struct BrickMap<VOX_F32_C> : compact::Map { typedef Vox<VOX_F32_C> V; };
 template <> struct BrickMap<VOX_F32_Q> : QuadMap<VOX_F32_Q> {};
 template <> struct BrickMap<VOX_U16_Q> : QuadMap<VOX_U16_Q> {};
 template <> struct BrickMap<VOX_U8_Q> : QuadMap<VOX_U8_Q> {};
@@ -339,6 +350,35 @@
     t.c001 = (float)q1.x; t.c101 = (float)q1.y; t.c011 = (float)q1.z; t.c111 = (float)q1.w;
     return;
   }
+  if constexpr (compact_layout(VT)) {
+    static_assert(AM <= 2, "the compact replica's tap reads the axis tables");
+    constexpr unsigned one = AM == 0 ? (unsigned)sizeof(T) : 1u;
+    const unsigned ox = vc.tab_x[t.x0], ox1 = vc.tab_x[t.x0 + 1];
+    const unsigned o0 = ox + vc.tab_y[t.y0], o1 = ox + vc.tab_y[t.y0 + 1];
+    const unsigned d = ox1 - ox;
+    typedef typename std::conditional<AM == 0, char, T>::type B;
+    const B* base = static_cast<const B*>(vc.data);
+    const B *r00, *r10, *r01, *r11;
+    if (AM == 2) {
+      const unsigned long long oz0 = vc.tab_z64[t.z0], oz1 = vc.tab_z64[t.z0 + 1];
+      r00 = base + (oz0 + o0); r10 = base + (oz0 + o1); r01 = base + (oz1 + o0); r11 = base + (oz1 + o1);
+    }
+    else {
+      const unsigned oz0 = vc.tab_z[t.z0], oz1 = vc.tab_z[t.z0 + 1];
+      r00 = base + (oz0 + o0); r10 = base + (oz0 + o1); r01 = base + (oz1 + o0); r11 = base + (oz1 + o1);
+    }
+    const P p00 = *reinterpret_cast<const P*>(r00), p10 = *reinterpret_cast<const P*>(r10);
+    const P p01 = *reinterpret_cast<const P*>(r01), p11 = *reinterpret_cast<const P*>(r11);
+    T u00 = 0, u10 = 0, u01 = 0, u11 = 0;
+    const bool straddle = d != one;
+    if (straddle) {
+      u00 = *reinterpret_cast<const T*>(r00 + d); u10 = *reinterpret_cast<const T*>(r10 + d);
+      u01 = *reinterpret_cast<const T*>(r01 + d); u11 = *reinterpret_cast<const T*>(r11 + d);
+    }
+    t.c000 = p00.x; t.c100 = straddle ? u00 : p00.y; t.c010 = p10.x; t.c110 = straddle ? u10 : p10.y;
+    t.c001 = p01.x; t.c101 = straddle ? u01 : p01.y; t.c011 = p11.x; t.c111 = straddle ? u11 : p11.y;
+    return;
+  }
   constexpr bool TR = Vox<VT>::kTransposed;
   const int a0 = TR ? t.y0 : t.x0, b0 = TR ? t.x0 : t.y0, z0 = t.z0;
   P p00, p10, p01, p11;
@@ -716,7 +756,7 @@
   const int na = Vox<VT>::kTransposed ? P.vol.ny : P.vol.nx, nb = Vox<VT>::kTransposed ? P.vol.nx : P.vol.ny;
   const unsigned int* __restrict__ gab = P.vol.axis_ab;
   const unsigned long long* __restrict__ gz = P.vol.axis_z;
-  const int ea = axis_a_entries(na), nab = ea + axis_b_entries(nb), ez = axis_z_entries(P.vol.nz);
+  const int ea = axis_a_entries(na, compact_layout(VT)), nab = ea + axis_b_entries(nb), ez = axis_z_entries(P.vol.nz);
   if (AM == 2) {
     unsigned long long* tz = reinterpret_cast<unsigned long long*>(base);
     unsigned int* tx = reinterpret_cast<unsigned int*>(tz + ez);
@@ -1001,7 +1041,7 @@
 template <int VT, int SHADE, int AM, bool POOLED, bool SKIP, bool LDSB = false, bool DEEP = false, bool MAT = false, bool CLIP = false, bool CACHED = false>
 __global__ __launch_bounds__(kBlock) __attribute__((amdgpu_waves_per_eu((SKIP && POOLED && (AM == 4 ? 0 : AM) <= kPinMaxAM) ? kMarchWavesPerEu : 1, kMarchWavesPerEu))) void raymarch_kernel(const RayMarchParams P)
 {
-  static_assert(march_variant_exists(SHADE, AM, POOLED, SKIP, LDSB, DEEP, MAT, CLIP, VT == VOX_F32, CACHED), "no such variant of the march (host/launch_plan.hpp)");
+  static_assert(march_variant_exists(SHADE, AM, POOLED, SKIP, LDSB, DEEP, MAT, CLIP, VT == VOX_F32, CACHED, compact_layout(VT)), "no such variant of the march (host/launch_plan.hpp)");
   using Cfg = QCfg<SHADE, POOLED>;
   constexpr int K = DEEP ? kDeepK : Cfg::K;
   constexpr int QCAP = Cfg::QCAP;
@@ -2375,9 +2415,26 @@
   return IsosurfaceKernels();
 }
 
+template <int VT, int SHADE>
+FrameKernel compact_march_of(int am)
+{
+  switch (am) {
+  case 0: return raymarch_kernel<VT, SHADE, 0, true, false>;
+  case 1: return raymarch_kernel<VT, SHADE, 1, true, false>;
+  case 2: return raymarch_kernel<VT, SHADE, 2, true, false>;
+  default: return nullptr;
+  }
+}
 template <int VT>
 FrameKernels frame_kernels(const LaunchPlan& pl)
 {
+  if constexpr (compact_layout(VT)) {
+    FrameKernels k;
+    if (pl.error || !pl.march.compact || !pl.pooled || pl.skip || pl.march.deep || pl.march.clipped) return k;
+    k.march = pl.shading == 1 ? compact_march_of<VT, 1>(pl.march.compact_am) : pl.shading == 2 ? compact_march_of<VT, 2>(pl.march.compact_am) : nullptr;
+    return k;
+  }
+  else {
   const unsigned flags = (pl.skip ? kBitSkip : 0u) | (pl.pooled ? kBitPooled : 0u) | (pl.march.lds_staged ? kBitLdsStaged : 0u) | (pl.march.deep ? kBitDeep : 0u);
   const unsigned march_bits = flags | (pl.march.material ? kBitMaterial : 0u) | (pl.march.clipped ? kBitClipped : 0u) | (pl.cached && !pl.pooled ? kBitCached : 0u);
   const unsigned shade_bits = (flags & kBitSkip) | (pl.shade.material ? kBitMaterial : 0u) | (pl.shade.clipped ? kBitClipped : 0u) | (pl.cached ? kBitCached : 0u);
@@ -2390,6 +2447,7 @@
   }
   if (!pl.pooled) k.shade = nullptr;
   return k;
-}
-
-}
+  }
+}
+
+}
diff --git a/open-volume-renderer_amd/csrc/ovr_hip_kernels.h b/open-volume-renderer_amd/csrc/ovr_hip_kernels.h
--- a/open-volume-renderer_amd/csrc/ovr_hip_kernels.h
+++ b/open-volume-renderer_amd/csrc/ovr_hip_kernels.h
@@ -9,9 +9,10 @@
 namespace ovrhip {
 
 enum VoxelType : int { VOX_U8 = 0, VOX_I8 = 1, VOX_U16 = 2, VOX_I16 = 3, VOX_F32 = 4, VOX_F32_T = 5, VOX_F32_TT = 6, VOX_U16_T = 7, VOX_U16_TT = 8, VOX_F32_Q = 9,
-                       VOX_U16_Q = 10, VOX_U8_Q = 11 };
-enum VolumeLayout : int { LAYOUT_GENERAL = 0, LAYOUT_THIN = 1, LAYOUT_THIN_T = 2, LAYOUT_QUAD = 3 };
+                       VOX_U16_Q = 10, VOX_U8_Q = 11, VOX_F32_C = 12 };
+enum VolumeLayout : int { LAYOUT_GENERAL = 0, LAYOUT_THIN = 1, LAYOUT_THIN_T = 2, LAYOUT_QUAD = 3, LAYOUT_COMPACT = 4 };
 constexpr int kLayouts = 4;
+constexpr int kReplicaSlots = 5;
 #define OVR_VOXEL_TYPES(X) \
   X(VOX_U8, u8, VOX_U8, LAYOUT_GENERAL) \
   X(VOX_I8, i8, VOX_I8, LAYOUT_GENERAL) \
@@ -24,7 +25,8 @@
   X(VOX_U16_TT, u16tt, VOX_U16, LAYOUT_THIN_T) \
   X(VOX_F32_Q, f32q, VOX_F32, LAYOUT_QUAD) \
   X(VOX_U16_Q, u16q, VOX_U16, LAYOUT_QUAD) \
-  X(VOX_U8_Q, u8q, VOX_U8, LAYOUT_QUAD)
+  X(VOX_U8_Q, u8q, VOX_U8, LAYOUT_QUAD) \
+  X(VOX_F32_C, f32c, VOX_F32, LAYOUT_COMPACT)
 struct VoxelTypeInfo { int type; const char* name; int base; int layout; };
 #define OVR_X(E, NAME, BASE, LAYOUT) { E, #NAME, BASE, LAYOUT },
 constexpr VoxelTypeInfo kVoxelTypes[] = { OVR_VOXEL_TYPES(OVR_X) };
@@ -36,7 +38,7 @@
     if (kVoxelTypes[i].type != i || kVoxelTypes[kVoxelTypes[i].base].layout != LAYOUT_GENERAL) return false;
   return true;
 }
-static_assert(kVoxelTypeCount == 12 && VOX_U8_Q == 11 && voxel_types_match_enum(), "the list restates the VoxelType enum: entry i is the type of value i");
+static_assert(kVoxelTypeCount == 13 && VOX_F32_C == 12 && voxel_types_match_enum(), "the list restates the VoxelType enum: entry i is the type of value i");
 template <bool GENERAL_ONLY = false, typename F>
 inline bool dispatch_voxel_type(int voxel_type, F&& f)
 {
@@ -59,6 +61,7 @@
 }
 constexpr int kBlockCounters = 8;
 
+constexpr bool compact_layout(int voxel_type) { return voxel_type == VOX_F32_C; }
 struct VolumeDesc {
   const void* data;
   int type;
@@ -71,7 +74,7 @@
   const unsigned int* axis_ab;
   const unsigned long long* axis_z;
 };
-__host__ __device__ constexpr int axis_a_entries(int na) { return na + 1; }
+__host__ __device__ constexpr int axis_a_entries(int na, bool compact = false) { return na + 1 + (compact ? 1 : 0); }
 __host__ __device__ constexpr int axis_b_entries(int nb) { return nb + 2; }
 __host__ __device__ constexpr int axis_z_entries(int nz) { return nz + 2; }
 
@@ -179,8 +182,8 @@
 hipError_t launch_shadow_cache(const RayMarchParams& p, const ShadowBuildArgs& a, hipStream_t stream);
 hipError_t launch_shadow_lookup(const RayMarchParams& p, const float* pos, float* out, int64_t n, hipStream_t stream);
 
-LaunchPlan plan_raymarch(const RayMarchParams& p);
-hipError_t launch_raymarch(const RayMarchParams& p, const LaunchPlan& plan, hipStream_t stream, const hipEvent_t* ev);
+LaunchPlan plan_raymarch(const RayMarchParams& p, const VolumeDesc* compact = nullptr, int compact_choice = -1);
+hipError_t launch_raymarch(const RayMarchParams& p, const LaunchPlan& plan, hipStream_t stream, const hipEvent_t* ev, const VolumeDesc* compact = nullptr);
 size_t pool_shade_blocks();
 size_t raymarch_lds_bytes(int n_color, int n_alpha);
 int volume_addressing_mode(const VolumeDesc& vd, int n_color, int n_alpha);
diff --git a/open-volume-renderer_amd/csrc/ovr_hip_kernels.hip b/open-volume-renderer_amd/csrc/ovr_hip_kernels.hip
--- a/open-volume-renderer_amd/csrc/ovr_hip_kernels.hip
+++ b/open-volume-renderer_amd/csrc/ovr_hip_kernels.hip
@@ -866,7 +866,7 @@
 
 size_t pool_shade_blocks() { return kShadeBlocks; }
 
-LaunchPlan plan_raymarch(const RayMarchParams& p)
+LaunchPlan plan_raymarch(const RayMarchParams& p, const VolumeDesc* compact, int compact_choice)
 {
   static const int deep = getenv("OVR_HIP_DEEP") ? atoi(getenv("OVR_HIP_DEEP")) : -1;
   static const int shade_blocks = getenv("OVR_HIP_SHADE_BLOCKS") ? atoi(getenv("OVR_HIP_SHADE_BLOCKS")) : 0;
@@ -892,6 +892,8 @@
   f.shadow_cache = p.shadow_lattice != nullptr;
   f.projection = p.projection; f.ranges = p.mc_ranges != nullptr;
   f.isosurfaces = p.iso_n;
+  if (compact && compact_layout(compact->type)) f.compact_bytes = compact->bytes;
+  o.compact = compact_choice;
   return plan_launch(f, o);
 }
 
@@ -903,7 +905,7 @@
   return hipSuccess;
 }
 
-static hipError_t launch_sequence(const RayMarchParams& p, const LaunchPlan& plan, const FrameKernels& k, hipStream_t stream, const hipEvent_t* ev)
+static hipError_t launch_sequence(const RayMarchParams& p, const LaunchPlan& plan, const FrameKernels& k, hipStream_t stream, const hipEvent_t* ev, const VolumeDesc* compact)
 {
   const dim3 grid((unsigned)raymarch_grid_blocks(p));
   hipError_t e;
@@ -931,7 +933,13 @@
   for (int g = 0; g < p.spp; ++g) {
     q.spp_index = g;
     if (g > 0 && (e = hipMemsetAsync(p.pool.ctrl, 0, (size_t)32 * (kPoolSubs + 1) * sizeof(unsigned int), stream)) != hipSuccess) return e;
-    if ((e = launch_variant(k.march, grid, plan.march_lds_bytes, stream, q)) != hipSuccess) return e;
+    if (plan.march.compact) {
+      RayMarchParams qm = q;
+      qm.vol = *compact;
+      qm.vol.value_scale = q.vol.value_scale; qm.vol.value_min_clamp = q.vol.value_min_clamp;
+      if ((e = launch_variant(k.march, grid, plan.march_lds_bytes, stream, qm)) != hipSuccess) return e;
+    }
+    else if ((e = launch_variant(k.march, grid, plan.march_lds_bytes, stream, q)) != hipSuccess) return e;
     if ((e = hipGetLastError()) != hipSuccess) return e;
     if (ev && ev[1] && g == p.spp - 1) (void)hipEventRecord(ev[1], stream);
     if (q.pool.order && (e = launch_shade_order(q, stream)) != hipSuccess) return e;
@@ -967,14 +975,16 @@
   return k;
 }
 
-hipError_t launch_raymarch(const RayMarchParams& p, const LaunchPlan& plan, hipStream_t stream, const hipEvent_t* ev)
+hipError_t launch_raymarch(const RayMarchParams& p, const LaunchPlan& plan, hipStream_t stream, const hipEvent_t* ev, const VolumeDesc* compact)
 {
   if (ev) (void)hipEventRecord(ev[0], stream);
   FrameKernels k;
   if (plan.isosurface.on) k.march = isosurface_kernels(p, plan).frame;
   else if (plan.project.mode != 0) k.march = project_kernels(p, plan).frame;
   else dispatch_voxel_type(p.vol.type, [&](auto vt) { k = frame_kernels<decltype(vt)::value>(plan); });
-  const hipError_t e = k.march && (k.shade || !plan.pooled) ? launch_sequence(p, plan, k, stream, ev) : hipErrorInvalidValue;
+  if (plan.march.compact && k.march)
+    k.march = compact && compact_layout(compact->type) && compact->data && compact->axis_ab && compact->axis_z ? frame_kernels<VOX_F32_C>(plan).march : nullptr;
+  const hipError_t e = k.march && (k.shade || !plan.pooled) ? launch_sequence(p, plan, k, stream, ev, compact) : hipErrorInvalidValue;
   if (ev) (void)hipEventRecord(ev[3], stream);
   return e;
 }
@@ -1196,7 +1206,7 @@
 {
   typedef BrickMap<VT> M;
   const int na = Vox<VT>::kTransposed ? ny : nx, nb = Vox<VT>::kTransposed ? nx : ny;
-  vd.macros_x = (na + 1 + (int)M::MCX - 1) / (int)M::MCX;
+  vd.macros_x = compact_layout(VT) ? compact::macros_x(na) : (na + 1 + (int)M::MCX - 1) / (int)M::MCX;
   vd.macros_y = ((Vox<VT>::kQuad ? nb + 1 : nb) + 31) / 32;
   vd.macros_z = (nz + 31) / 32;
   vd.macro_elems = M::MV;
@@ -1228,6 +1238,8 @@
   typedef typename Vox<VTB>::T T;
   typedef SrcBricked<VTB> Src;
   constexpr int T1 = replica_voxel_type(VTB, LAYOUT_THIN), T2 = replica_voxel_type(VTB, LAYOUT_THIN_T), TQ = replica_voxel_type(VTB, LAYOUT_QUAD);
+  constexpr int TC = replica_voxel_type(VTB, LAYOUT_COMPACT);
+  if constexpr (TC >= 0) { if (vd.type == TC) return relayout_s<Src, T, TC>(src_bricked<VTB>(g), dst, vd, z0, nzc, stream); }
   if constexpr (TQ >= 0) { if (vd.type == TQ) return relayout_quad_s<Src, TQ>(src_bricked<VTB>(g), dst, vd, z0, nzc, stream); }
   if constexpr (T1 >= 0) { if (vd.type == T1) return relayout_s<Src, T, T1>(src_bricked<VTB>(g), dst, vd, z0, nzc, stream); }
   if constexpr (T2 >= 0) { if (vd.type == T2) return relayout_s<Src, T, T2>(src_bricked<VTB>(g), dst, vd, z0, nzc, stream); }
@@ -1334,6 +1346,7 @@
 {
   typedef Vox<VT> V;
   update::Geometry g{ V::cx, V::mbx, V::by, V::bz, V::kTransposed, V::kQuad, 0, 0, 0 };
+  g.apron = compact_layout(VT) ? 0 : 1;
   if constexpr (V::kQuad) { g.lx = V::lx; g.ly = V::ly; g.lz = V::lz; }
   return g;
 }
@@ -1382,6 +1395,8 @@
   typedef typename Vox<VTB>::T T;
   typedef SrcBricked<VTB> Src;
   constexpr int T1 = replica_voxel_type(VTB, LAYOUT_THIN), T2 = replica_voxel_type(VTB, LAYOUT_THIN_T), TQ = replica_voxel_type(VTB, LAYOUT_QUAD);
+  constexpr int TC = replica_voxel_type(VTB, LAYOUT_COMPACT);
+  if constexpr (TC >= 0) { if (vd.type == TC) return update_rows_s<Src, T, TC>(src_bricked<VTB>(g), dst, vd, box, stream); }
   if constexpr (TQ >= 0) { if (vd.type == TQ) return update_quad_s<Src, TQ>(src_bricked<VTB>(g), dst, vd, box, stream); }
   if constexpr (T1 >= 0) { if (vd.type == T1) return update_rows_s<Src, T, T1>(src_bricked<VTB>(g), dst, vd, box, stream); }
   if constexpr (T2 >= 0) { if (vd.type == T2) return update_rows_s<Src, T, T2>(src_bricked<VTB>(g), dst, vd, box, stream); }
@@ -1402,8 +1417,9 @@
   const unsigned int macro_y = macro_stride_y(vd);
   const unsigned long long macro_z = macro_stride_z(vd);
   const int i = (int)(blockIdx.x * 256u + threadIdx.x);
-  if (i < axis_a_entries(na)) ab[i] = M::X((unsigned)i);
-  if (i < axis_b_entries(nb)) ab[axis_a_entries(na) + i] = M::Y(Vox<VT>::kQuad ? (unsigned)min(i, nb) : (unsigned)min(max(i - 1, 0), nb - 1), macro_y);
+  constexpr bool C = compact_layout(VT);
+  if (i < axis_a_entries(na, C)) ab[i] = M::X((unsigned)i);
+  if (i < axis_b_entries(nb)) ab[axis_a_entries(na, C) + i] = M::Y(Vox<VT>::kQuad ? (unsigned)min(i, nb) : (unsigned)min(max(i - 1, 0), nb - 1), macro_y);
   if (i < axis_z_entries(vd.nz)) {
     const unsigned z = (unsigned)min(max(i - 1, 0), vd.nz - 1);
     tz[i] = (unsigned long long)M::Zlo(z) + (unsigned long long)(z >> 5) * macro_z;
@@ -1411,7 +1427,7 @@
 }
 size_t axis_table_bytes(const VolumeDesc& vd)
 {
-  return (size_t)axis_z_entries(vd.nz) * sizeof(unsigned long long) + (size_t)(vd.nx + vd.ny + 3) * sizeof(unsigned int);
+  return (size_t)axis_z_entries(vd.nz) * sizeof(unsigned long long) + (size_t)(vd.nx + vd.ny + 3 + (compact_layout(vd.type) ? 1 : 0)) * sizeof(unsigned int);
 }
 template <int VT>
 static hipError_t axis_tables_t(const VolumeDesc& vd, unsigned int* ab, unsigned long long* tz, hipStream_t stream)
```

After: 97580, median of 4. 1.04x the previous value.
